# feiyeha/BS-YOLO

Hardware: AMD Instinct MI355X
Metric: images/sec YOLO11s 640x640 bs=64 (forward + NMS) (higher is better)
Workload: dtype f16

## Files before the change

### bs_yolo_amd/csrc/common.h

```cpp
#pragma once
#include <hip/hip_runtime.h>
#include <stdint.h>
#include <stdio.h>
#include <string>

#include "../../include/bsyolo.h"

typedef _Float16 half_t;
typedef _Float16 half8 __attribute__((ext_vector_type(8)));
typedef _Float16 half4 __attribute__((ext_vector_type(4)));
typedef _Float16 half2v __attribute__((ext_vector_type(2)));
typedef float f32x16 __attribute__((ext_vector_type(16)));
typedef float f32x4 __attribute__((ext_vector_type(4)));

void bsy_set_error(const char* fmt, ...);
#define BSY_FAIL(code, ...)        \
    do {                           \
        bsy_set_error(__VA_ARGS__); \
        return (code);             \
    } while (0)
#define HIP_TRY(expr)                                                                                     \
    do {                                                                                                  \
        hipError_t _e = (expr);                                                                           \
        if (_e != hipSuccess) BSY_FAIL(BSY_ERR_HIP, "%s failed: %s (%s:%d)", #expr, hipGetErrorString(_e), \
                                       __FILE__, __LINE__);                                               \
    } while (0)

static inline int ceil_div(int a, int b) { return (a + b - 1) / b; }
static inline int round_up(int a, int b) { return ceil_div(a, b) * b; }

struct ConvArgs {
    const half_t* src0;
    const half_t* src1;
    int ld0, ld1;
    int C0, C1;
    int up0, up1;
    int B, H, W, OH, OW;
    int ksize, stride, pad;
    const half_t* wgt;
    const float* bias;
    void* dst;
    int ldd, Cout, out_f32;
    const half_t* res;
    int ldr;
    int act;
    int dst_scale, dst_dy, dst_dx;
    int cfg;
    int epi;
    void* y;
    int y_f32, A, a0, nrows;
    float lvl_stride;
    void* raw;
    int raw_f32, rawC;
    const half_t* tail_wgt;
    const float* tail_bias;
    int nsl_c = 0, nsl_t = 0;
    float* split_ws = nullptr;
};
int launch_conv(const ConvArgs& a, hipStream_t s);
#define BSY_CONV_MAX_CFG 64
int conv_candidates(const ConvArgs& a, int* out, int max_out);
bool conv_cfg_valid(const ConvArgs& a, int cfg);
int conv_korder(const ConvArgs& a);

struct ConvFirstArgs {
    const void* img;
    int img_dtype;
    int B, H, W, OH, OW, ksize, stride, pad;
    const void* w;
    const float* b;
    half_t* dst;
    int ldd, Cout, act;
};
int launch_conv_first(const ConvFirstArgs& a, hipStream_t s);

struct StemArgs {
    const void* img;
    int img_dtype;
    int B, H, W, OH, OW;
    const void* w0;
    const float* b0;
    const void* w1;
    const float* b1;
    int C0, C1, Kpad1;
    half_t* dst;
    int ldd, act;
};
bool stem_fused_supported(int C0, int C1, int H, int W);
int launch_stem_fused(const StemArgs& a, hipStream_t s);

struct BneckArgs {
    const half_t* src;
    int lds;
    int B, H, W, C, CH;
    const void *w1, *w2;
    const float *b1, *b2;
    int Kpad1, Kpad2;
    half_t* dst;
    int ldd, act;
};
bool bneck_fused_supported(int C, int CH);
int launch_bneck_fused(const BneckArgs& a, hipStream_t s);

struct C3k2Args {
    const half_t* src;
    int lds;
    int B, H, W, Cin, C, C2;
    const void *w1, *wa, *wb, *w4;
    const float *b1, *ba, *bb, *b4;
    half_t* dst;
    int ldd;
};
bool c3k2_fused_supported(int Cin, int C, int C2);
int launch_c3k2_fused(const C3k2Args& a, hipStream_t s);

struct DwGenArgs {
    const half_t* src;
    int lds;
    int B, H, W, C, OH, OW, kh, kw, stride;
    const float* w;
    int wld;
    const float* b;
    half_t* dst;
    int ldd, act_c;
    int ident_c0 = 0;
};
int launch_dwconv_generic(const DwGenArgs& a, hipStream_t s);
struct PmsfaArgs {
    const half_t* P;
    int ldp;
    const half_t* x;
    int ldx;
    half_t* dst;
    int ldd;
    int B, H, W, C;
    const float* w2;
    const float* b2;
    int wld2;
    const float* w3;
    const float* b3;
// ... 290 lines not shown
```

### bs_yolo_amd/csrc/conv_gemm.hip

```cpp
#include "conv_kernels.h"


__device__ __attribute__((aligned(16))) unsigned int bsy_zero_page[16];

template <int KS, int WAVES_M, int WAVES_N, int MT, int NT, int STAGES, bool ALIGNED, int BK>
__global__ __launch_bounds__(64 * WAVES_M * WAVES_N) void conv_mfma_kernel(const ConvK p) {
    constexpr int NW = WAVES_M * WAVES_N;
    constexpr int NTHR = 64 * NW;
    static_assert(BK == 32 || (BK == 64 && ALIGNED), "BK = 64 only for aligned layers");
    constexpr int TM = WAVES_M * MT * 32;
    constexpr int TN = WAVES_N * NT * 32;
    constexpr int TNS = TN < 64 ? 64 : TN;
    constexpr int CPR = BK / 8;
    constexpr int RPI = 64 / CPR;
    constexpr int PIW = TM / (RPI * NW);
    constexpr int WIW = TNS / (RPI * NW);
    static_assert(PIW >= 1 && WIW >= 1 && (BK == 32 || (!(PIW & 1) && !(WIW & 1))), "tile too small for this wave count");
    constexpr int STAGE = (TM + TNS) * BK;
    constexpr int NDMA = PIW + WIW;
    constexpr int SWS = BK == 32 ? 2 : 1;
    constexpr int OTILE = (TM > TN ? TM : TN) * ((TM > TN ? TN : TM) + 8);
    constexpr int SMEM = STAGES * STAGE > OTILE ? STAGES * STAGE : OTILE;
    __shared__ __attribute__((aligned(16))) half_t smem[SMEM];

    const int tid = threadIdx.x;
    const int lane = tid & 63;
    const int wave = __builtin_amdgcn_readfirstlane(tid >> 6);
    const int wm = wave / WAVES_N, wn = wave % WAVES_N;
    int wg = xcd_remap(blockIdx.x, gridDim.x);
    const bool split = ALIGNED && p.nsl_c * p.nsl_t > 1;
    int slice = 0;
    if (split) {
        const int per = p.ntn * ((p.M + TM - 1) / TM);
        slice = wg / per;
        wg -= slice * per;
    }
    const int tap0 = split ? (slice % p.nsl_t) * p.taps_per : 0, tap1 = split ? tap0 + p.taps_per : p.ntaps;
    const int cb0 = split ? (slice / p.nsl_t) * p.cb_per : 0, cb1 = split ? cb0 + p.cb_per : p.Cin8 * 8;
    const int tn_idx = wg % p.ntn;
    const int tm_idx = wg / p.ntn;
    const int m0 = tm_idx * TM;
    const int n0 = tn_idx * TN;

    const int rsub = lane / CPR;
    const int slot = lane % CPR;
    const int kc0 = BK == 32 ? (slot ^ ((rsub >> 2) & 3)) : (slot ^ (rsub >> 1));
    const int kc1 = BK == 32 ? kc0 : (slot ^ (4 | (rsub >> 1)));
    unsigned off0[PIW], off1[PIW], vmask[PIW];
    const int ohw = p.OH * p.OW;
#pragma unroll
    for (int i = 0; i < PIW; ++i) {
        const int m = m0 + (wave * PIW + i) * RPI + rsub;
        const bool rv = m < p.M;
        const int mm = rv ? m : 0;
        int n, oh, ow;
        if (KS == 1 && p.stride == 1) {
            n = 0; oh = 0; ow = 0;
            if (p.up0 | p.up1) { n = mm / ohw; const int rem = mm - n * ohw; oh = rem / p.OW; ow = rem - oh * p.OW; }
        } else {
            n = mm / ohw; const int rem = mm - n * ohw; oh = rem / p.OW; ow = rem - oh * p.OW;
        }
        const int iy0 = oh * p.stride - p.pad, ix0 = ow * p.stride - p.pad;
        if (KS == 1) {
            vmask[i] = rv ? 1u : 0u;
            if (p.stride == 1 && !(p.up0 | p.up1)) {
                off0[i] = (unsigned)mm * (unsigned)p.ld0;
                off1[i] = (unsigned)mm * (unsigned)p.ld1;
            } else {
                const int H0 = p.H >> p.up0, W0 = p.W >> p.up0, H1 = p.H >> p.up1, W1 = p.W >> p.up1;
                off0[i] = (unsigned)((n * H0 + (iy0 >> p.up0)) * W0 + (ix0 >> p.up0)) * (unsigned)p.ld0;
                off1[i] = (unsigned)((n * H1 + (iy0 >> p.up1)) * W1 + (ix0 >> p.up1)) * (unsigned)p.ld1;
            }
        } else {
            unsigned rb = 0, cb = 0;
#pragma unroll
            for (int t = 0; t < KS; ++t) {
                rb |= ((unsigned)(iy0 + t) < (unsigned)p.H ? 1u : 0u) << t;
                cb |= ((unsigned)(ix0 + t) < (unsigned)p.W ? 1u : 0u) << t;
            }
            unsigned vm = 0;
#pragma unroll
            for (int t = 0; t < KS; ++t) vm |= ((rb >> t) & 1u) ? (cb << (t * KS)) : 0u;
            vmask[i] = rv ? vm : 0u;
            const unsigned pix = (unsigned)((n * p.H + iy0) * p.W + ix0);
            off0[i] = pix * (unsigned)p.ld0;
            off1[i] = pix * (unsigned)p.ld1;
        }
    }
    unsigned woff[WIW];
#pragma unroll
    for (int j = 0; j < WIW; ++j)
    {
        const int wrow = min(n0 + (wave * WIW + j) * RPI + rsub, ((p.Cout + 127) & ~127) - 1);
        woff[j] = (unsigned)wrow * (unsigned)p.Kpad + ((j & 1) ? kc1 : kc0) * 8;
    }
    const half_t* zero = reinterpret_cast<const half_t*>(bsy_zero_page);
    const bsy_rsrc_t rs0 = make_rsrc(p.src0, p.span0), rs1 = make_rsrc(p.src1 ? p.src1 : p.src0, p.src1 ? p.span1 : 0u),
                     rsw = make_rsrc(p.wgt, p.wspan);

    int s_tap = tap0, s_cb = cb0;
    int tap = ALIGNED ? 0 : kc0 / p.Cin8;
    int c8 = ALIGNED ? 0 : kc0 - tap * p.Cin8;
    const int Cin = p.Cin8 * 8;

    auto issue = [&](int kt, int stage, const int s_tap, const int s_cb, const int tap, const int c8) {
        half_t* sP = smem + stage * STAGE;
        half_t* sW = sP + TM * BK;
#ifdef BSY_ABLATE
        if (BSY_ABLATE & 1) return;
#endif
        if (ALIGNED) {
            const bool s1 = s_cb >= p.C0;
            const int ld = s1 ? p.ld1 : p.ld0;
            const int kh = (KS == 1) ? 0 : s_tap / KS;
            const int kw = (KS == 1) ? 0 : s_tap - kh * KS;
            const unsigned sc = 2u * (unsigned)((kh * p.W + kw) * ld + (s1 ? s_cb - p.C0 : s_cb));
            const unsigned tbit = 1u << s_tap;
#pragma unroll
            for (int i = 0; i < PIW; ++i) {
                const unsigned kcb = 16u * (unsigned)((i & 1) ? kc1 : kc0);
                const unsigned o = (vmask[i] & tbit) ? 2u * (s1 ? off1[i] : off0[i]) + sc + kcb : BSY_OOB;
                if (s1) dma16_buf(rs1, o, 0u, sP + (wave * PIW + i) * RPI * BK);
                else dma16_buf(rs0, o, 0u, sP + (wave * PIW + i) * RPI * BK);
            }
#pragma unroll
            for (int j = 0; j < WIW; ++j)
                dma16_buf(rsw, 2u * woff[j], 2u * (unsigned)(s_tap * Cin + s_cb), sW + (wave * WIW + j) * RPI * BK);
        } else {
            const bool kvalid = tap < p.ntaps;
            const int kh = (KS == 1) ? 0 : tap / KS;
            const int kw = (KS == 1) ? 0 : tap - kh * KS;
            const int cc = c8 * 8;
            const bool s1 = cc >= p.C0;
            const half_t* base = s1 ? p.src1 : p.src0;
            const int ld = s1 ? p.ld1 : p.ld0;
            const unsigned sc = (unsigned)((kh * p.W + kw) * ld + (s1 ? cc - p.C0 : cc));
            const unsigned tbit = kvalid ? (1u << tap) : 0u;
#pragma unroll
            for (int i = 0; i < PIW; ++i) {
                const unsigned o = (s1 ? off1[i] : off0[i]) + sc;
                const half_t* g = (vmask[i] & tbit) ? base + (size_t)o : zero;
                dma16(g, sP + (wave * PIW + i) * RPI * BK);
            }
#pragma unroll
            for (int j = 0; j < WIW; ++j)
                dma16(p.wgt + (size_t)(woff[j] + (unsigned)kt * 32u), sW + (wave * WIW + j) * RPI * BK);
        }
    };
#define BSY_ADVANCE_K()                                                                                  \
    do {                                                                                                 \
        if (ALIGNED) {                                                                                   \
            if (p.korder == 1 || (p.korder == 2 && BK == 64)) {  \
                if (++s_tap >= tap1) { s_tap = tap0; s_cb += BK; }                                       \
            } else if (p.korder == 2) {        \
                if (s_cb & 32) { s_cb -= 32; if (++s_tap >= tap1) { s_tap = tap0; s_cb += 64; } }        \
                else s_cb += 32;                                                                         \
            } else {                                                                                     \
                s_cb += BK;                                                                              \
                if (s_cb >= cb1) { s_cb = cb0; ++s_tap; }                                                \
            }                                                                                            \
        } else {                                                                                         \
            c8 += 4;                                                                                     \
            while (c8 >= p.Cin8) { c8 -= p.Cin8; ++tap; }                                                \
        }                                                                                                \
    } while (0)

    const int lrow = lane & 31;
    const int lh = lane >> 5;
    const int nk = split ? (tap1 - tap0) * (cb1 - cb0) / BK : p.Kpad / BK;
    f32x16 acc[NT][MT];
#pragma unroll
    for (int a = 0; a < NT; ++a)
#pragma unroll
        for (int b = 0; b < MT; ++b) {
            acc_bias(acc[a][b], p.bias + n0 + (wn * NT + a) * 32, lh);
            if (slice) {
#pragma unroll
                for (int r = 0; r < 16; ++r) acc[a][b][r] = 0.f;
            }
        }

#pragma unroll
    for (int s = 0; s < STAGES - 1; ++s)
        if (s < nk) { issue(s, s, s_tap, s_cb, tap, c8); BSY_ADVANCE_K(); }

    for (int kt = 0; kt < nk; ++kt) {
        const int later = min(STAGES - 2, nk - 1 - kt);
        if (later >= STAGES - 2 && STAGES > 2) {
            asm volatile("s_waitcnt vmcnt(%0)" ::"n"((STAGES - 2) * NDMA) : "memory");
        } else if (STAGES > 3 && later == STAGES - 3) {
            asm volatile("s_waitcnt vmcnt(%0)" ::"n"((STAGES > 3 ? STAGES - 3 : 0) * NDMA) : "memory");
        } else {
            asm volatile("s_waitcnt vmcnt(0)" ::: "memory");
        }
        __builtin_amdgcn_s_barrier();
        if (kt + STAGES - 1 < nk) { issue(kt + STAGES - 1, (kt + STAGES - 1) % STAGES, s_tap, s_cb, tap, c8); BSY_ADVANCE_K(); }
        const half_t* sP = smem + (kt % STAGES) * STAGE;
        const half_t* sW = sP + TM * BK;
        constexpr int KSUB = BK / 16;
        half8 bfr[2][MT], afr[2][NT];
        auto rd = [&](const int ks, const int buf) {
            const int chunk = 2 * ks + lh;
#pragma unroll
            for (int b = 0; b < MT; ++b) {
                const int row = (wm * MT + b) * 32 + lrow;
                bfr[buf][b] = *reinterpret_cast<const half8*>(sP + row * BK + ((chunk ^ ((row >> SWS) & (CPR - 1))) << 3));
            }
#pragma unroll
            for (int a = 0; a < NT; ++a) {
                const int row = (wn * NT + a) * 32 + lrow;
                afr[buf][a] = *reinterpret_cast<const half8*>(sW + row * BK + ((chunk ^ ((row >> SWS) & (CPR - 1))) << 3));
            }
        };
        rd(0, 0);
#pragma unroll
        for (int ks = 0; ks < KSUB; ++ks) {
            if (ks + 1 < KSUB) rd(ks + 1, (ks + 1) & 1);
            __builtin_amdgcn_sched_barrier(0);
#pragma unroll
            for (int a = 0; a < NT; ++a)
#pragma unroll
                for (int b = 0; b < MT; ++b)
                    acc[a][b] = __builtin_amdgcn_mfma_f32_32x32x16_f16(afr[ks & 1][a], bfr[ks & 1][b], acc[a][b], 0, 0, 0);
            __builtin_amdgcn_sched_barrier(0);
        }
    }
#ifdef BSY_ABLATE
    if (BSY_ABLATE & 4) {
        if (acc[0][0][0] == 12345.678f) reinterpret_cast<float*>(p.dst)[0] = 1.f;
        return;
    }
#endif
    if (split) {
        float* ws = p.split_ws + (size_t)slice * (size_t)p.slab;
#pragma unroll
        for (int b = 0; b < MT; ++b) {
            const int m = m0 + (wm * MT + b) * 32 + lrow;
            if (m >= p.M) continue;
#pragma unroll
            for (int a = 0; a < NT; ++a) {
                const int cbase = n0 + (wn * NT + a) * 32;
#pragma unroll
                for (int g = 0; g < 4; ++g) {
                    const int c = cbase + 8 * g + 4 * lh;
                    if (c < p.ldw) *reinterpret_cast<f32x4*>(ws + (size_t)m * p.ldw + c) = f32x4{acc[a][b][4 * g], acc[a][b][4 * g + 1], acc[a][b][4 * g + 2], acc[a][b][4 * g + 3]};
                }
            }
        }
        return;
    }
    if (p.epi) {
        if (p.epi == 2 && !p.y_f32 && !p.raw) {
            __syncthreads();
            conv_epilogue_cls_lds<TM, TN, MT, NT, NTHR>(p, acc, smem, m0, n0, wm, wn, lrow, lh, tid);
        } else {
            conv_epilogue_head<MT, NT>(p, acc, m0, n0, wm, wn, lrow, lh);
        }
        return;
    }
    const bool lds_epi = !p.out_f32 && !(p.Cout & 7) && !(p.ldd & 7) && !((uintptr_t)p.dst & 15) && p.dst_scale == 1 &&
                         (!p.res || (!(p.ldr & 7) && !((uintptr_t)p.res & 15)));
    if (lds_epi) {
        __syncthreads();
        conv_epilogue_lds<TM, TN, MT, NT, NTHR>(p, acc, smem, m0, n0, wm, wn, lrow, lh, tid);
    } else {
        conv_epilogue<MT, NT>(p, acc, m0, n0, wm, wn, lrow, lh);
    }
}

#undef BSY_ADVANCE_K

__global__ __launch_bounds__(256) void splitk_reduce_kernel(const float* __restrict__ ws, const int nsl, const long long slab, const int ldw,
                                                           const int M, const int Cout, const int act, const half_t* __restrict__ res, const int ldr,
                                                           half_t* __restrict__ dst, const int ldd) {
    const int c8n = Cout >> 3;
    const long long idx = (long long)blockIdx.x * 256 + threadIdx.x;
    if (idx >= (long long)M * c8n) return;
    const int c = (int)(idx % c8n) * 8;
    const size_t m = (size_t)(idx / c8n);
    const float* wp = ws + m * ldw + c;
    f32x4 a0 = *reinterpret_cast<const f32x4*>(wp), a1 = *reinterpret_cast<const f32x4*>(wp + 4);
    for (int sl = 1; sl < nsl; ++sl) {
        const float* q = wp + (size_t)sl * (size_t)slab;
        a0 = add4_f(a0, *reinterpret_cast<const f32x4*>(q));
        a1 = add4_f(a1, *reinterpret_cast<const f32x4*>(q + 4));
    }
    float v[8] = {a0[0], a0[1], a0[2], a0[3], a1[0], a1[1], a1[2], a1[3]};
    if (act) {
#pragma unroll
        for (int e = 0; e < 8; ++e) v[e] = silu_f(v[e]);
    }
    if (res) {
        const half8 rv = *reinterpret_cast<const half8*>(res + m * ldr + c);
#pragma unroll
        for (int e = 0; e < 8; ++e) v[e] += (float)rv[e];
    }
    half8 o;
#pragma unroll
    for (int e = 0; e < 8; ++e) o[e] = (half_t)v[e];
    *reinterpret_cast<half8*>(dst + m * ldd + c) = o;
}

template <int KS, int WM, int WN, int MT, int NT, int STAGES, bool ALIGNED, int BK>
static int launch_cfg(const ConvK& k, hipStream_t s) {
    constexpr int TM = WM * MT * 32, TN = WN * NT * 32;
    ConvK p = k;
    p.ntn = ceil_div(k.Cout, TN);
    const int nsl = k.nsl_c * k.nsl_t;
    const long long nblk = (long long)ceil_div(k.M, TM) * p.ntn * (nsl > 1 ? nsl : 1);
    if (nblk <= 0 || nblk > 0x7fffffffLL) BSY_FAIL(BSY_ERR_ARG, "conv: grid %lld out of range", nblk);
    hipLaunchKernelGGL((conv_mfma_kernel<KS, WM, WN, MT, NT, STAGES, ALIGNED, BK>), dim3((unsigned)nblk), dim3(64 * WM * WN), 0, s, p);
    HIP_TRY(hipGetLastError());
    if (nsl > 1) {
        const long long items = (long long)k.M * (k.Cout >> 3);
        hipLaunchKernelGGL(splitk_reduce_kernel, dim3((unsigned)((items + 255) / 256)), dim3(256), 0, s, k.split_ws, nsl, k.slab, k.ldw, k.M, k.Cout, k.act,
                           k.res, k.ldr, reinterpret_cast<half_t*>(k.dst), k.ldd);
        HIP_TRY(hipGetLastError());
    }
    return BSY_OK;
}

template <int WM, int WN, int MT, int NT, int S, bool AL, int BK>
static int launch_gemm(int ksize, const ConvK& k, hipStream_t s) {
    return ksize == 3 ? launch_cfg<3, WM, WN, MT, NT, S, AL, BK>(k, s) : launch_cfg<1, WM, WN, MT, NT, S, AL, BK>(k, s);
}

int launch_gemm_cfg(int id, int ksize, const ConvK& k, hipStream_t s) {
    switch (id) {
        case 0x00: return launch_gemm<4, 1, 2, 1, 3, false, 32>(ksize, k, s);
        case 0x01: return launch_gemm<4, 1, 2, 1, 3, true, 32>(ksize, k, s);
        case 0x02: return launch_gemm<4, 1, 2, 1, 2, true, 32>(ksize, k, s);
        case 0x03: return launch_gemm<4, 1, 2, 1, 2, true, 64>(ksize, k, s);
        case 0x10: return launch_gemm<4, 1, 2, 2, 3, false, 32>(ksize, k, s);
        case 0x11: return launch_gemm<4, 1, 2, 2, 3, true, 32>(ksize, k, s);
        case 0x12: return launch_gemm<4, 1, 2, 2, 2, true, 32>(ksize, k, s);
        case 0x13: return launch_gemm<4, 1, 2, 2, 2, true, 64>(ksize, k, s);
        case 0x20: return launch_gemm<2, 2, 2, 2, 3, false, 32>(ksize, k, s);
        case 0x21: return launch_gemm<2, 2, 2, 2, 3, true, 32>(ksize, k, s);
        case 0x22: return launch_gemm<2, 2, 2, 2, 2, true, 32>(ksize, k, s);
        case 0x23: return launch_gemm<2, 2, 2, 2, 2, true, 64>(ksize, k, s);
        case 0x30: return launch_gemm<2, 2, 2, 1, 3, false, 32>(ksize, k, s);
        case 0x31: return launch_gemm<2, 2, 2, 1, 3, true, 32>(ksize, k, s);
        case 0x32: return launch_gemm<2, 2, 2, 1, 2, true, 32>(ksize, k, s);
        case 0x33: return launch_gemm<2, 2, 2, 1, 2, true, 64>(ksize, k, s);
        case 0x41: return launch_gemm<4, 2, 2, 2, 3, true, 32>(ksize, k, s);
        case 0x42: return launch_gemm<4, 2, 2, 2, 2, true, 32>(ksize, k, s);
        case 0x43: return launch_gemm<4, 2, 2, 2, 2, true, 64>(ksize, k, s);
        case 0x50: return launch_gemm<1, 4, 2, 1, 3, false, 32>(ksize, k, s);
        case 0x51: return launch_gemm<1, 4, 2, 1, 3, true, 32>(ksize, k, s);
        case 0x52: return launch_gemm<1, 4, 2, 1, 2, true, 32>(ksize, k, s);
        case 0x53: return launch_gemm<1, 4, 2, 1, 2, true, 64>(ksize, k, s);
        case 0x60: return launch_gemm<2, 2, 1, 1, 3, false, 32>(ksize, k, s);
        case 0x61: return launch_gemm<2, 2, 1, 1, 3, true, 32>(ksize, k, s);
        case 0x62: return launch_gemm<2, 2, 1, 1, 2, true, 32>(ksize, k, s);
        case 0x63: return launch_gemm<2, 2, 1, 1, 2, true, 64>(ksize, k, s);
        case 0x71: return launch_gemm<4, 2, 2, 4, 3, true, 32>(ksize, k, s);
        case 0x72: return launch_gemm<4, 2, 2, 4, 2, true, 32>(ksize, k, s);
        case 0x73: return launch_gemm<4, 2, 2, 4, 2, true, 64>(ksize, k, s);
    }
    BSY_FAIL(BSY_ERR_ARG, "conv: no implicit-GEMM kernel is built for configuration 0x%02x", id);
}
```

### bs_yolo_amd/csrc/conv_kernels.h

```cpp
#pragma once
#include "common.h"

struct ConvK {
    const half_t* src0;
    const half_t* src1;
    int ld0, ld1, C0, C1, up0, up1;
    int H, W, OH, OW, stride, pad;
    int M;
    int Cin8;
    int ntaps;
    int nk;
    int Kpad;
    const half_t* wgt;
    const float* bias;
    void* dst;
    int ldd, Cout, out_f32;
    const half_t* res;
    int ldr;
    int act;
    int dst_scale, dst_dy, dst_dx;
    int ntn;
    int ntm;
    int tiles_x, tiles_y, B;
    int epi, y_f32, A, a0, nrows, raw_f32, rawC;
    float lvl_stride;
    void* y;
    void* raw;
    const half_t* tail_wgt;
    const float* tail_bias;
    unsigned span0, span1, wspan;
    int nsl_c, nsl_t, cb_per, taps_per, ldw;
    float* split_ws;
    long long slab;
    int korder;
};

__device__ __forceinline__ void dma16(const void* g, half_t* lds_wave_base) {
#if defined(__HIP_DEVICE_COMPILE__)
    __builtin_amdgcn_global_load_lds(g, lds_wave_base, 16, 0, 0);
#else
    (void)g;
    (void)lds_wave_base;
#endif
}

#if defined(__HIP_DEVICE_COMPILE__)
__device__ __forceinline__ void dma16_buf(bsy_rsrc_t r, unsigned voff, unsigned soff, half_t* lds_wave_base) {
    __builtin_amdgcn_raw_ptr_buffer_load_lds(r, lds_wave_base, 16, (int)voff, (int)soff, 0, 0);
}
#else
__device__ __forceinline__ void dma16_buf(bsy_rsrc_t, unsigned, unsigned, half_t*) {}
#endif

template <int MT, int NT>
__device__ __forceinline__ void conv_epilogue(const ConvK& p, f32x16 (&acc)[NT][MT], int m0, int n0, int wm, int wn,
                                              int lrow, int lh) {
    const int ohw = p.OH * p.OW;
    const bool wide = !p.out_f32 && !(p.Cout & 15) && !(p.ldd & 7) && !((uintptr_t)p.dst & 15);
#pragma unroll
    for (int b = 0; b < MT; ++b) {
        const int m = m0 + (wm * MT + b) * 32 + lrow;
        const bool mvalid = m < p.M;
        size_t dpix = (size_t)(mvalid ? m : 0);
        if (p.dst_scale != 1) {
            const int mm = mvalid ? m : 0;
            const int n = mm / ohw;
            const int rem = mm - n * ohw;
            const int oh = rem / p.OW;
            const int ow = rem - oh * p.OW;
            dpix = ((size_t)n * (p.OH * p.dst_scale) + (oh * p.dst_scale + p.dst_dy)) * (size_t)(p.OW * p.dst_scale) +
                   (ow * p.dst_scale + p.dst_dx);
        }
#pragma unroll
        for (int a = 0; a < NT; ++a) {
            const int cbase = n0 + (wn * NT + a) * 32;
            if (cbase >= p.Cout) continue;
            if (wide) {
                unsigned pk[4][2];
#pragma unroll
                for (int g = 0; g < 4; ++g) {
                    const int c = cbase + 8 * g + 4 * lh;
                    float v[4] = {0.f, 0.f, 0.f, 0.f};
                    if (c < p.Cout) {
#pragma unroll
                        for (int e = 0; e < 4; ++e) {
                            float t = acc[a][b][4 * g + e];
                            v[e] = p.act ? silu_f(t) : t;
                        }
                        if (p.res && mvalid) {
                            const half4 rv = *reinterpret_cast<const half4*>(p.res + dpix * p.ldr + c);
#pragma unroll
                            for (int e = 0; e < 4; ++e) v[e] += (float)rv[e];
                        }
                    }
                    half2v h0 = {(half_t)v[0], (half_t)v[1]}, h1 = {(half_t)v[2], (half_t)v[3]};
                    pk[g][0] = __builtin_bit_cast(unsigned, h0);
                    pk[g][1] = __builtin_bit_cast(unsigned, h1);
                }
#pragma unroll
                for (int g = 0; g < 4; g += 2) {
                    const auto r0 = __builtin_amdgcn_permlane32_swap(pk[g][0], pk[g + 1][0], false, false);
                    const auto r1 = __builtin_amdgcn_permlane32_swap(pk[g][1], pk[g + 1][1], false, false);
                    const int c = cbase + 8 * (g + lh);
                    if (mvalid && c < p.Cout) {
                        uint4 o = {r0[0], r1[0], r0[1], r1[1]};
                        *reinterpret_cast<uint4*>(reinterpret_cast<half_t*>(p.dst) + dpix * p.ldd + c) = o;
                    }
                }
                continue;
            }
            if (!mvalid) continue;
#pragma unroll
            for (int g = 0; g < 4; ++g) {
                const int c = cbase + 8 * g + 4 * lh;
                if (c >= p.Cout) continue;
                float v[4];
#pragma unroll
// ... 138 lines not shown
                                                      int wm, int wn, int lrow, int lh, int tid) {
    constexpr int LDP = TM + 8;
#pragma unroll
    for (int b = 0; b < MT; ++b) {
        const int prow = (wm * MT + b) * 32 + lrow;
#pragma unroll
        for (int a = 0; a < NT; ++a) {
            const int cl = (wn * NT + a) * 32;
            if (n0 + cl >= p.Cout) continue;
#pragma unroll
            for (int g = 0; g < 4; ++g) {
                const int c = cl + 8 * g + 4 * lh;
#pragma unroll
                for (int e = 0; e < 4; ++e) {
                    const float v = acc[a][b][4 * g + e];
                    stile[(c + e) * LDP + prow] = (half_t)sigmoid_f(v);
                }
            }
        }
    }
    __syncthreads();
    const int hw = p.OH * p.OW;
    half_t* y = reinterpret_cast<half_t*>(p.y);
    constexpr int GPR = TM / 8;
    for (int id = tid; id < TN * GPR; id += NTHR) {
        const int cr = id / GPR, g8 = (id - cr * GPR) * 8;
        const int c = n0 + cr, m = m0 + g8;
        if (c >= p.Cout || m >= p.M) continue;
        const int n = m / hw, pix = m - n * hw;
        const size_t yi = ((size_t)n * p.nrows + 4 + c) * p.A + p.a0 + pix;
        if (pix + 8 <= hw && m + 8 <= p.M && !(yi & 7)) {
            *reinterpret_cast<half8*>(y + yi) = *reinterpret_cast<const half8*>(stile + cr * LDP + g8);
        } else {
            for (int e = 0; e < 8 && m + e < p.M; ++e) {
                const int me = m + e, ne = me / hw, pe = me - ne * hw;
                y[((size_t)ne * p.nrows + 4 + c) * p.A + p.a0 + pe] = stile[cr * LDP + g8 + e];
            }
        }
    }
}

template <int TM, int TN, int MT, int NT, int NTHR>
__device__ __forceinline__ void conv_epilogue_lds(const ConvK& p, f32x16 (&acc)[NT][MT], half_t* stile, int m0, int n0,
                                                  int wm, int wn, int lrow, int lh, int tid) {
    constexpr int LDT = TN + 8;
#pragma unroll
    for (int b = 0; b < MT; ++b) {
        const int prow = (wm * MT + b) * 32 + lrow;
#pragma unroll
        for (int a = 0; a < NT; ++a) {
            const int cl = (wn * NT + a) * 32;
#pragma unroll
            for (int g = 0; g < 4; ++g) {
                const int c = cl + 8 * g + 4 * lh;
                half4 o;
                f32x4 t = f32x4{acc[a][b][4 * g], acc[a][b][4 * g + 1], acc[a][b][4 * g + 2], acc[a][b][4 * g + 3]};
                if (p.act) t = silu4_f(t);
#pragma unroll
                for (int e = 0; e < 4; ++e) o[e] = (half_t)t[e];
                *reinterpret_cast<half4*>(stile + prow * LDT + c) = o;
            }
        }
    }
    __syncthreads();
    constexpr int CPRW = TN / 8;
    constexpr int ITER = TM * CPRW / NTHR;
    half_t* dst = reinterpret_cast<half_t*>(p.dst);
#pragma unroll
    for (int i = 0; i < ITER; ++i) {
        const int id = tid + NTHR * i;
        const int row = id / CPRW, cc = (id % CPRW) * 8;
        const int m = m0 + row, c = n0 + cc;
        if (m >= p.M || c >= p.Cout) continue;
        half8 v = *reinterpret_cast<const half8*>(stile + row * LDT + cc);
        if (p.res) {
            const half8 r = *reinterpret_cast<const half8*>(p.res + (size_t)m * p.ldr + c);
#pragma unroll
            for (int e = 0; e < 8; ++e) v[e] = (half_t)((float)v[e] + (float)r[e]);
        }
        *reinterpret_cast<half8*>(dst + (size_t)m * p.ldd + c) = v;
    }
}

int launch_gemm_cfg(int id, int ksize, const ConvK& k, hipStream_t s);
int launch_stream1x1_cfg(int id, const ConvK& k, hipStream_t s);
int launch_patch_cfg(int id, bool tail, const ConvK& k, hipStream_t s);

constexpr int PERSIST_MAX_COUT = 1024;
```

### bs_yolo_amd/csrc/conv_select.hip

```cpp
#include <stdlib.h>

#include "conv_kernels.h"

extern "C" int bsy_conv_packed_dims(int C2, int C1, int ksize, int* cout_pad, int* k_pad) {
    if (C2 <= 0 || C1 <= 0 || (ksize != 1 && ksize != 3)) BSY_FAIL(BSY_ERR_ARG, "conv_packed_dims: bad shape");
    if (cout_pad) *cout_pad = round_up(C2, 128);
    if (C1 == 3) C1 = 4;
    if (k_pad) *k_pad = round_up(ksize * ksize * C1, 32);
    return BSY_OK;
}

int conv_korder(const ConvArgs& a) {
    const int Cin = a.C0 + a.C1;
    if (a.ksize != 3 || (Cin & 31) || (a.C0 & 31)) return 0;
    return (a.stride == 2 && !(Cin & 63) && !(a.C0 & 63)) ? 2 : 1;
}

enum ConvFam { CONV_GEMM, CONV_PERSIST, CONV_WRES, CONV_PATCH, CONV_TAIL };
struct ConvCfg {
    int id; ConvFam fam;
    int tm, tn, stages, bk;
    bool aligned;
    int tw, nfr;
};
template <int WM, int WN, int MT, int NT, int S, bool AL, int BK> constexpr ConvCfg gemm_row(int id) {
    return {id, CONV_GEMM, WM * MT * 32, WN * NT * 32, S, BK, AL, 0, 0};
}
template <int WM, int WN, int MT, int NT, int S, int BK> constexpr ConvCfg persist_row(int id) {
    return {id, CONV_PERSIST, WM * MT * 32, WN * NT * 32, S, BK, true, 0, 0};
}
template <int NT, int S, int NFR> constexpr ConvCfg wres_row(int id) {
    return {id, CONV_WRES, 128, 64 * NT, S, 32, true, 0, NFR};
}
template <int NT, int S, int TW, bool TAIL = false> constexpr ConvCfg patch_row(int id) {
    return {id, TAIL ? CONV_TAIL : CONV_PATCH, TW == 16 ? 8 * 16 : 6 * 20, 64 * NT, S, 32, true, TW, 0};
}
static const ConvCfg kConvCfgs[] = {
    gemm_row<4, 1, 2, 1, 3, false, 32>(0x00),
    gemm_row<4, 1, 2, 1, 3, true, 32>(0x01),
    gemm_row<4, 1, 2, 1, 2, true, 32>(0x02),
    gemm_row<4, 1, 2, 1, 2, true, 64>(0x03),
    gemm_row<4, 1, 2, 2, 3, false, 32>(0x10),
    gemm_row<4, 1, 2, 2, 3, true, 32>(0x11),
    gemm_row<4, 1, 2, 2, 2, true, 32>(0x12),
    gemm_row<4, 1, 2, 2, 2, true, 64>(0x13),
    gemm_row<2, 2, 2, 2, 3, false, 32>(0x20),
    gemm_row<2, 2, 2, 2, 3, true, 32>(0x21),
    gemm_row<2, 2, 2, 2, 2, true, 32>(0x22),
    gemm_row<2, 2, 2, 2, 2, true, 64>(0x23),
    gemm_row<2, 2, 2, 1, 3, false, 32>(0x30),
    gemm_row<2, 2, 2, 1, 3, true, 32>(0x31),
    gemm_row<2, 2, 2, 1, 2, true, 32>(0x32),
    gemm_row<2, 2, 2, 1, 2, true, 64>(0x33),
    gemm_row<4, 2, 2, 2, 3, true, 32>(0x41),
    gemm_row<4, 2, 2, 2, 2, true, 32>(0x42),
    gemm_row<4, 2, 2, 2, 2, true, 64>(0x43),
    gemm_row<1, 4, 2, 1, 3, false, 32>(0x50),
    gemm_row<1, 4, 2, 1, 3, true, 32>(0x51),
    gemm_row<1, 4, 2, 1, 2, true, 32>(0x52),
    gemm_row<1, 4, 2, 1, 2, true, 64>(0x53),
    gemm_row<2, 2, 1, 1, 3, false, 32>(0x60),
    gemm_row<2, 2, 1, 1, 3, true, 32>(0x61),
    gemm_row<2, 2, 1, 1, 2, true, 32>(0x62),
    gemm_row<2, 2, 1, 1, 2, true, 64>(0x63),
    gemm_row<4, 2, 2, 4, 3, true, 32>(0x71),
    gemm_row<4, 2, 2, 4, 2, true, 32>(0x72),
    gemm_row<4, 2, 2, 4, 2, true, 64>(0x73),
    persist_row<2, 2, 2, 2, 3, 32>(0x81),
    persist_row<2, 2, 2, 2, 2, 32>(0x82),
    persist_row<2, 2, 2, 2, 2, 64>(0x83),
    persist_row<2, 2, 2, 1, 3, 32>(0x91),
    persist_row<2, 2, 2, 1, 2, 32>(0x92),
    persist_row<2, 2, 2, 1, 2, 64>(0x93),
    patch_row<2, 2, 16>(0xA1),
    patch_row<1, 3, 16>(0xB1),
    patch_row<1, 2, 16>(0xB2),
    patch_row<1, 4, 16>(0xB3),
    patch_row<2, 2, 20>(0xC1),
    patch_row<1, 3, 20>(0xD1),
    patch_row<1, 2, 20>(0xD2),
    patch_row<1, 4, 20>(0xD3),
    patch_row<1, 3, 16, true>(0xB1),
    patch_row<1, 2, 16, true>(0xB2),
    patch_row<1, 4, 16, true>(0xB3),
    patch_row<1, 3, 20, true>(0xD1),
    patch_row<1, 2, 20, true>(0xD2),
    patch_row<1, 4, 20, true>(0xD3),
    wres_row<2, 4, 24>(0xE1),
    wres_row<2, 3, 24>(0xE2),
    wres_row<1, 4, 32>(0xF1),
    wres_row<1, 3, 32>(0xF2),
};

static const ConvCfg* conv_cfg_row(int cfg, bool tail) {
    for (const ConvCfg& r : kConvCfgs) if (r.id == (cfg & ~4) && (r.fam == CONV_TAIL) == tail) return &r;
    return nullptr;
}

bool conv_cfg_valid(const ConvArgs& a, int cfg) {
    const ConvCfg* r = conv_cfg_row(cfg, a.tail_wgt != nullptr);
    if (!r) return false;
    const int Cin = a.C0 + a.C1, ko = conv_korder(a), nsl = a.nsl_c * a.nsl_t;
    const bool aligned = !(Cin & 31) && !(a.C0 & 31), aligned64 = !(Cin & 63) && !(a.C0 & 63);
    if ((r->aligned && !aligned) || (r->bk == 64 && !aligned64)) return false;
    if (r->fam == CONV_GEMM) {
        if (!(cfg & 4) != !ko) return false;
        if (ko && (!r->aligned || (ko == 1 && r->bk == 64))) return false;
        if (nsl > 1 && (!r->aligned || (Cin / (a.nsl_c > 0 ? a.nsl_c : 1)) % r->bk)) return false;
        if (a.epi == 3 && (r->tm != 256 || r->tn != 64)) return false;
        return r->tn != 256 || !(a.Cout & 255);
    }
    if ((cfg & 4) || nsl > 1 || (r->fam == CONV_TAIL ? (a.epi != 3 || a.Cout != 64 || a.res) : a.epi != 0)) return false;
    if (a.out_f32 || (a.Cout & 7) || (a.ldd & 7) || ((uintptr_t)a.dst & 15) || a.dst_scale > 1) return false;
    if (r->fam == CONV_PERSIST || r->fam == CONV_WRES) {
        if (a.ksize != 1 || a.stride != 1 || a.res) return false;
        if (r->fam == CONV_PERSIST) return a.Cout <= PERSIST_MAX_COUT;
        return (r->tn / 64) * (Cin / 16) <= r->nfr && Cin / 32 >= r->stages - 1 && (r->tn != 128 || a.Cout > 64);
    }
    return ko == 1 && a.ksize == 3 && a.stride == 1 && a.pad == 1 && !a.C1 && !a.up0 && (!a.res || (!(a.ldr & 7) && !((uintptr_t)a.res & 15))) &&
           (r->tn != 128 || a.Cout > 64);
}

static bool family_off(const char* env) { return getenv(env) != nullptr; }

int conv_candidates(const ConvArgs& a, int* out, int max_out) {
    const int Cin = a.C0 + a.C1;
    const bool aligned = !(Cin & 31) && !(a.C0 & 31), aligned64 = !(Cin & 63) && !(a.C0 & 63);
    const long long M = (long long)a.B * a.OH * a.OW;
    const int tile = a.epi == 3 ? 1 : (a.Cout > 64 ? 2 : (a.Cout > 32 ? 1 : 0));
    const int ko = conv_korder(a), km = ko ? 4 : 0;
    const bool t20 = ceil_div(a.W, 20) * ceil_div(a.H, 6) < ceil_div(a.W, 16) * ceil_div(a.H, 8);
    int n = 0;
    auto add = [&](int c) {
        for (int i = 0; i < n; ++i) if (out[i] == c) return;
        if (n < max_out && conv_cfg_valid(a, c)) out[n++] = c;
    };
    if (a.tail_wgt) {
        if (t20) { add(0xD2); add(0xD1); add(0xD3); }
        add(0xB2); add(0xB1); add(0xB3); add(0xD2); add(0xD1); add(0xD3);
        return n;
    }
    if (!aligned) {
        add(tile << 4);
        if (a.Cout > 32) { add(0x30); add(0x60); }
        if (a.Cout > 64) add(0x50);
        return n;
    }
    const bool patch_ok = !family_off("BSY_NO_PATCH");
    if (!a.epi && a.ksize == 3 && a.stride == 1 && a.H >= 16 && a.W >= 16 && patch_ok) add(t20 ? 0xD2 : 0xB2);
    const int vbest = (aligned64 && ko != 1) ? 3 : 1;
    if (!a.epi && !(a.Cout & 255) && aligned64 && ko != 1 && M >= 16384) add(0x73 | km);
    add(tile << 4 | vbest | km);
    for (const ConvCfg& r : kConvCfgs) {
        if ((r.fam != CONV_GEMM && r.fam != CONV_PERSIST) || !r.aligned) continue;
        if (r.tn >= 2 * round_up(a.Cout, 32)) continue;
        if (r.tn == 32 && a.Cout > 32) continue;
        if (r.tm == 256 && r.tn == 128 && (a.Cout < 128 || M < 32768)) continue;
        if (r.tn == 256 && M < 16384) continue;
        if (r.fam == CONV_PERSIST && (M < 65536 || family_off("BSY_NO_PERSIST"))) continue;
        add(r.id | (r.fam == CONV_GEMM ? km : 0));
    }
    if (a.ksize == 1 && M >= 65536 && !family_off("BSY_NO_WRES"))
        for (const ConvCfg& r : kConvCfgs) if (r.fam == CONV_WRES) add(r.id);
    if (a.H >= 16 && a.W >= 16 && patch_ok)
        for (const ConvCfg& r : kConvCfgs) if (r.fam == CONV_PATCH && (r.tw == 16 || t20)) add(r.id);
    return n;
}

int launch_conv(const ConvArgs& a, hipStream_t s) {
    const int Cin = a.C0 + a.C1;
    if (a.ksize != 1 && a.ksize != 3) BSY_FAIL(BSY_ERR_ARG, "conv: ksize %d unsupported", a.ksize);
    if (a.stride != 1 && a.stride != 2) BSY_FAIL(BSY_ERR_ARG, "conv: stride %d unsupported", a.stride);
    if ((a.C0 & 7) || (a.C1 & 7) || (a.ld0 & 7) || (a.C1 && (a.ld1 & 7)))
        BSY_FAIL(BSY_ERR_ARG, "conv: channel counts/strides must be multiples of 8 (C0=%d C1=%d ld0=%d ld1=%d)", a.C0,
                 a.C1, a.ld0, a.ld1);
    if ((a.ldd & 3) || (a.res && (a.ldr & 3))) BSY_FAIL(BSY_ERR_ARG, "conv: dst/res row stride must be a multiple of 4");
    if (((uintptr_t)a.src0 & 15) || ((uintptr_t)a.src1 & 15) || ((uintptr_t)a.wgt & 15) || ((uintptr_t)a.bias & 15) ||
        ((uintptr_t)a.dst & 7) || ((uintptr_t)a.res & 7))
        BSY_FAIL(BSY_ERR_ARG, "conv: misaligned pointer");
    if (a.C1 && !a.src1) BSY_FAIL(BSY_ERR_ARG, "conv: src1 missing");
    if ((a.up0 && ((a.H | a.W) & 1)) || (a.up1 && ((a.H | a.W) & 1))) BSY_FAIL(BSY_ERR_ARG, "conv: odd size with upsample");
    if (a.OH != (a.H + 2 * a.pad - a.ksize) / a.stride + 1 || a.OW != (a.W + 2 * a.pad - a.ksize) / a.stride + 1)
        BSY_FAIL(BSY_ERR_ARG, "conv: output extent mismatch");
    const long long M = (long long)a.B * a.OH * a.OW;
    if (M <= 0 || M > 0x7fffffffLL) BSY_FAIL(BSY_ERR_ARG, "conv: M out of range");
    if (a.epi) {
        if ((a.epi != 2 && a.epi != 3) || !a.y || a.A <= 0 || a.a0 < 0 || a.a0 + a.OH * a.OW > a.A || a.dst_scale > 1 || a.res)
            BSY_FAIL(BSY_ERR_ARG, "conv: bad fused-decoder arguments (epi %d)", a.epi);
        if (a.epi == 3 && (a.Cout != 64 || a.nrows < 4)) BSY_FAIL(BSY_ERR_ARG, "conv: DFL epilogue needs 64 box channels");
        if (a.tail_wgt && (a.epi != 3 || !a.tail_bias || a.ksize != 3 || ((uintptr_t)a.tail_wgt & 15) || ((uintptr_t)a.tail_bias & 15)))
            BSY_FAIL(BSY_ERR_ARG, "conv: bad box-branch tail arguments");
        if (a.epi == 2 && a.nrows < 4 + a.Cout) BSY_FAIL(BSY_ERR_ARG, "conv: y has %d rows, class epilogue needs %d", a.nrows, 4 + a.Cout);
        if (a.raw && a.rawC < (a.epi == 3 ? 64 : 64 + a.Cout)) BSY_FAIL(BSY_ERR_ARG, "conv: raw map has too few channels");
    }
    ConvK k;
    k.src0 = a.src0; k.src1 = a.src1; k.ld0 = a.ld0; k.ld1 = a.ld1; k.C0 = a.C0; k.C1 = a.C1;
    k.up0 = a.up0; k.up1 = a.up1; k.H = a.H; k.W = a.W; k.OH = a.OH; k.OW = a.OW; k.stride = a.stride; k.pad = a.pad;
    k.M = (int)M; k.Cin8 = Cin / 8; k.ntaps = a.ksize * a.ksize;
    k.Kpad = round_up(a.ksize * a.ksize * Cin, 32); k.nk = k.Kpad / 32;
    k.wgt = a.wgt; k.bias = a.bias; k.dst = a.dst; k.ldd = a.ldd; k.Cout = a.Cout; k.out_f32 = a.out_f32;
    k.res = a.res; k.ldr = a.ldr; k.act = a.act; k.B = a.B; k.tiles_x = k.tiles_y = 0;
    k.epi = a.epi; k.y = a.y; k.y_f32 = a.y_f32; k.A = a.A; k.a0 = a.a0; k.nrows = a.nrows; k.lvl_stride = a.lvl_stride;
    k.raw = a.raw; k.raw_f32 = a.raw_f32; k.rawC = a.rawC;
    k.tail_wgt = a.tail_wgt; k.tail_bias = a.tail_bias;
    if (a.tail_wgt && !a.epi) BSY_FAIL(BSY_ERR_ARG, "conv: a box-branch tail needs the decoder arguments (epi 3)");
    k.dst_scale = a.dst_scale > 0 ? a.dst_scale : 1; k.dst_dy = a.dst_dy; k.dst_dx = a.dst_dx; k.ntn = 1;
    k.nsl_c = k.nsl_t = 1; k.cb_per = Cin; k.taps_per = a.ksize * a.ksize; k.split_ws = nullptr; k.slab = 0; k.ldw = 0;
    if (a.nsl_c * a.nsl_t > 1) {
        const int nt = a.ksize * a.ksize;
        if (a.nsl_c < 1 || a.nsl_t < 1 || !a.split_ws || a.epi || a.out_f32 || a.tail_wgt || (a.dst_scale > 1) || (Cin % a.nsl_c) || ((Cin / a.nsl_c) & 31) || (a.C0 & 31) ||
            (nt % a.nsl_t) || (a.Cout & 7) || (a.ldd & 7) || ((uintptr_t)a.dst & 15) || (a.res && ((a.ldr & 7) || ((uintptr_t)a.res & 15))) || ((uintptr_t)a.split_ws & 15))
            BSY_FAIL(BSY_ERR_ARG, "conv: bad split-K arguments (%d x %d slices)", a.nsl_c, a.nsl_t);
        if (conv_korder(a) == 2 && ((Cin / a.nsl_c) & 63)) BSY_FAIL(BSY_ERR_ARG, "conv: split-K slices of a 64-channel-chunk layer must be multiples of 64 channels");
        k.nsl_c = a.nsl_c; k.nsl_t = a.nsl_t; k.cb_per = Cin / a.nsl_c; k.taps_per = nt / a.nsl_t; k.split_ws = a.split_ws;
        k.ldw = round_up(a.Cout, 32);
        k.slab = (long long)M * k.ldw;
    }
    if (a.ksize == 3 && (a.up0 || a.up1)) BSY_FAIL(BSY_ERR_ARG, "conv: upsampled source only with ksize 1");
    if ((long long)a.B * a.H * a.W * (long long)(a.ld0 > a.ld1 ? a.ld0 : a.ld1) >= (1LL << 31))
        BSY_FAIL(BSY_ERR_ARG, "conv: source view exceeds 2^31 elements (split the batch)");
    {
        const long long px0 = (long long)a.B * (a.H >> a.up0) * (a.W >> a.up0), px1 = (long long)a.B * (a.H >> a.up1) * (a.W >> a.up1);
        k.span0 = (unsigned)(((px0 - 1) * a.ld0 + a.C0) * 2);
        k.span1 = a.C1 ? (unsigned)(((px1 - 1) * a.ld1 + a.C1) * 2) : 0u;
        k.wspan = (unsigned)((long long)round_up(a.Cout, 128) * k.Kpad * 2);
    }
    int cfg = a.cfg;
    if (cfg < 0 || !conv_cfg_valid(a, cfg)) {
        int list[BSY_CONV_MAX_CFG];
        if (conv_candidates(a, list, BSY_CONV_MAX_CFG) <= 0) BSY_FAIL(BSY_ERR_ARG, "conv: no kernel configuration for this shape");
        cfg = list[0];
    }
    k.korder = conv_korder(a);
    const ConvCfg* r = conv_cfg_row(cfg, a.tail_wgt != nullptr);
    switch (r->fam) {
        case CONV_GEMM: return launch_gemm_cfg(r->id, a.ksize, k, s);
        case CONV_PERSIST:
        case CONV_WRES: return launch_stream1x1_cfg(r->id, k, s);
        case CONV_PATCH:
        case CONV_TAIL: return launch_patch_cfg(r->id, r->fam == CONV_TAIL, k, s);
    }
    BSY_FAIL(BSY_ERR_ARG, "conv: configuration 0x%02x has no kernel family", cfg);
}
```

### bs_yolo_amd/csrc/engine.hip

```cpp
#include <stdlib.h>
#include <string.h>

#include <algorithm>
#include <vector>

#include "common.h"
#include "postproc.h"

struct bsy_engine {
    int device = 0;
    void* weights = nullptr;
    size_t weight_bytes = 0;
    char* arena = nullptr;
    size_t arena_bytes = 0;
    unsigned arena_gen = 0;
    unsigned weights_gen = 0;
};

struct bsy_plan {
    bsy_engine* eng = nullptr;
    std::vector<bsy_op> ops;
    std::vector<size_t> buf_off;
    std::vector<size_t> buf_size;
    char* workspace = nullptr;
// ... 416 lines not shown
            return launch_pmsfa_tail(a, s);
        }
        case BSY_OP_COPY: {
            const half_t* src = R.h(op.src0);
            half_t* dst = R.h(op.dst);
            if (!R.ok) return BSY_ERR_ARG;
            return launch_copy_view(src, op.src0.ld, op.up0, op.B, op.H, op.W, op.src0.C, dst, op.dst.ld, s);
        }
        case BSY_OP_GAP: {
            const half_t* src = R.h(op.src0);
            half_t* dst = R.h(op.dst);
            if (!R.ok) return BSY_ERR_ARG;
            return launch_gap(src, op.src0.ld, op.B, op.H, op.W, op.src0.C, dst, op.dst.ld, s);
        }
        case BSY_OP_MSCA_SPATIAL: {
            MscaSpArgs a;
            a.src = R.h(op.src0); a.lds = op.src0.ld; a.B = op.B; a.H = op.H; a.W = op.W; a.C = op.src0.C;
            for (int i = 0; i < 9; ++i) {
                a.w[i] = (const float*)(wb + op.aux_off[2 * i]);
                a.b[i] = (const float*)(wb + op.aux_off[2 * i + 1]);
            }
            for (int i = 0; i < 4; ++i) {
                const bsy_view& bv = i < 3 ? op.box[i] : op.res;
                const bsy_view& gv = i < 3 ? op.cls[i] : op.msk[0];
                a.br[i] = R.h(bv); a.ldb[i] = bv.ld; a.gap[i] = R.h(gv); a.ldg[i] = gv.ld;
            }
            if (!R.ok) return BSY_ERR_ARG;
            return launch_msca_spatial(a, s);
        }
        case BSY_OP_MSCA_MIX: {
            MixArgs a;
            for (int i = 0; i < 4; ++i) {
                const bsy_view& bv = i < 3 ? op.box[i] : op.res;
                const bsy_view& lv = i < 3 ? op.cls[i] : op.msk[0];
                a.br[i] = R.h(bv); a.ldb[i] = bv.ld; a.lg[i] = R.f(lv); a.ldl[i] = lv.ld;
            }
            a.B = op.B; a.HW = op.H * op.W; a.C = op.dst.C; a.dst = R.h(op.dst); a.ldd = op.dst.ld;
            if (!R.ok) return BSY_ERR_ARG;
            return launch_msca_mix(a, s);
        }
        case BSY_OP_MUL: {
            const half_t* x = R.h(op.src0);
            const half_t* y = R.h(op.src1);
            half_t* dst = R.h(op.dst);
            if (!R.ok) return BSY_ERR_ARG;
            return launch_mul(x, op.src0.ld, y, op.src1.ld, (long long)op.B * op.H * op.W, op.dst.C, dst, op.dst.ld, s);
        }
        case BSY_OP_ELA: {
            ElaArgs a;
            a.src = R.h(op.src0); a.lds = op.src0.ld; a.B = op.B; a.H = op.H; a.W = op.W; a.C = op.src0.C; a.k = op.ksize;
            const float* blob = (const float*)(wb + op.w_off);
            a.wsp = blob; a.wch = blob + (size_t)a.C * a.k; a.gnw = a.wch + (size_t)a.C * a.k; a.gnb = a.gnw + a.C;
            a.ch_coef = op.scale; a.sp_coef = op.lvl_stride[0]; a.res_coef = op.lvl_stride[1];
            a.scratch = R.f(op.res); a.dst = R.h(op.dst); a.ldd = op.dst.ld;
            if (!R.ok) return BSY_ERR_ARG;
            return launch_ela(a, s);
        }
        case BSY_OP_CONV: {
            ConvArgs a;
            a.src0 = R.h(op.src0); a.src1 = R.h(op.src1);
            a.ld0 = op.src0.ld; a.ld1 = op.src1.buf >= 0 ? op.src1.ld : 0;
            a.C0 = op.src0.C; a.C1 = op.src1.buf >= 0 ? op.src1.C : 0;
            a.up0 = op.up0; a.up1 = op.up1;
            a.B = op.B; a.H = op.H; a.W = op.W; a.OH = op.OH; a.OW = op.OW;
            a.ksize = op.ksize; a.stride = op.stride; a.pad = op.pad;
            a.wgt = (const half_t*)(wb + op.w_off); a.bias = (const float*)(wb + op.b_off);
            a.dst = op.out_f32 ? (void*)R.f(op.dst) : (void*)R.h(op.dst);
            a.ldd = op.dst.ld; a.Cout = op.dst.C; a.out_f32 = op.out_f32;
            a.res = R.h(op.res); a.ldr = op.res.buf >= 0 ? op.res.ld : 0;
            a.act = op.act; a.dst_scale = op.dst_scale; a.dst_dy = op.dst_dy; a.dst_dx = op.dst_dx;
            a.epi = 0; a.y = nullptr; a.raw = nullptr; a.y_f32 = a.raw_f32 = a.A = a.a0 = a.nrows = a.rawC = 0; a.lvl_stride = 0.f;
            a.tail_wgt = nullptr; a.tail_bias = nullptr;
            if (op.out_f32 >= 2) {
                a.epi = op.out_f32; a.out_f32 = 0; a.dst = nullptr; a.ldd = 8; a.Cout = op.nl;
                a.y = R.base(op.dst); a.y_f32 = op.out_dtype == BSY_F32; a.A = op.A; a.a0 = op.lvl_h[1]; a.nrows = op.dst.C;
                a.lvl_stride = op.lvl_stride[0];
                const bsy_view& rv = op.box[0];
                const bool bound = rv.buf >= BSY_EXT_BASE && rv.buf - BSY_EXT_BASE < R.n_ext && R.ext[rv.buf - BSY_EXT_BASE];
                a.raw = bound ? R.base(rv) : nullptr; a.raw_f32 = a.y_f32; a.rawC = rv.C;
                if (op.out_f32 == 3 && op.mid_c > 0) {
                    a.Cout = op.mid_c;
                    a.tail_wgt = (const half_t*)(wb + op.w2_off); a.tail_bias = (const float*)(wb + op.b2_off);
                }
            }
            if (op.ksplit > 0 && op.out_f32 == 0) {
                a.nsl_c = op.ksplit & 255; a.nsl_t = (op.ksplit >> 8) & 255;
                a.split_ws = R.f(op.box[0]);
            }
            a.cfg = op.tuned_cfg - 1;
            if (!R.ok) return BSY_ERR_ARG;
            if (cargs) { *cargs = a; return BSY_OK; }
            return launch_conv(a, s);
        }
        case BSY_OP_DWCONV: {
            DwArgs a;
            a.src = R.h(op.src0); a.lds = op.src0.ld; a.B = op.B; a.H = op.H; a.W = op.W; a.C = op.src0.C;
            a.w = (const float*)(wb + op.w_off); a.b = (const float*)(wb + op.b_off);
            a.dst = R.h(op.dst); a.ldd = op.dst.ld; a.act = op.act;
            a.res = R.h(op.res); a.ldr = op.res.buf >= 0 ? op.res.ld : 0;
            if (!R.ok) return BSY_ERR_ARG;
            return launch_dwconv(a, s);
        }
        case BSY_OP_SPPF_POOL: {
            half_t* b = R.h(op.src0);
            if (!R.ok) return BSY_ERR_ARG;
            return launch_sppf_pool(b, op.src0.ld, op.B, op.H, op.W, op.src0.C, s);
        }
        case BSY_OP_ATTN: {
            AttnArgs a;
            a.qkv = R.h(op.src0); a.ld = op.src0.ld; a.B = op.B; a.N = op.H * op.W; a.heads = op.heads;
            a.key_dim = op.key_dim; a.head_dim = op.head_dim; a.scale = op.scale;
            a.out = R.h(op.dst); a.ldo = op.dst.ld;
            if (!R.ok) return BSY_ERR_ARG;
            return launch_attention(a, s);
        }
        case BSY_OP_DECODE: {
            DecodeArgs a;
            memset(&a, 0, sizeof(a));
            a.nl = op.nl; a.B = op.B; a.nc = op.nc; a.nm = op.nm; a.A = op.A; a.ne = op.ne;
            const bool extra = op.nm || op.ne;
            for (int l = 0; l < op.nl && l < BSY_MAX_LEVELS; ++l) {
                a.box[l] = R.f(op.box[l]); a.cls[l] = R.f(op.cls[l]); a.msk[l] = extra ? R.f(op.msk[l]) : nullptr;
                a.ldb[l] = op.box[l].ld; a.ldc[l] = op.cls[l].ld; a.ldm[l] = extra ? op.msk[l].ld : 0;
                a.h[l] = op.lvl_h[l]; a.w[l] = op.lvl_w[l]; a.stride[l] = op.lvl_stride[l];
            }
            a.y = R.base(op.dst); a.y_dtype = op.out_dtype;
            if (!R.ok) return BSY_ERR_ARG;
            return launch_decode(a, s);
        }
        case BSY_OP_RAW_NCHW: {
            const int l = op.level;
            if (l < 0 || l >= BSY_MAX_LEVELS) BSY_FAIL(BSY_ERR_ARG, "raw_nchw: level %d", l);
            if (op.dst.buf >= BSY_EXT_BASE && (op.dst.buf - BSY_EXT_BASE >= R.n_ext || !R.ext[op.dst.buf - BSY_EXT_BASE]))
                return BSY_OK;
            const float* box = R.f(op.box[l]);
            const float* cls = R.f(op.cls[l]);
            void* out = R.base(op.dst);
            if (!R.ok) return BSY_ERR_ARG;
            return launch_raw_nchw(box, op.box[l].ld, cls, op.cls[l].ld, op.B, op.lvl_h[l], op.lvl_w[l], op.nc, out,
                                   op.out_dtype, s);
        }
        case BSY_OP_NHWC2NCHW: {
            if (op.dst.buf >= BSY_EXT_BASE && (op.dst.buf - BSY_EXT_BASE >= R.n_ext || !R.ext[op.dst.buf - BSY_EXT_BASE]))
                return BSY_OK;
            const half_t* src = R.h(op.src0);
            void* out = R.base(op.dst);
            if (!R.ok) return BSY_ERR_ARG;
            return launch_nhwc2nchw(src, op.src0.ld, op.B, op.src0.C, op.H * op.W, out, op.out_dtype, s);
        }
        default:
            BSY_FAIL(BSY_ERR_ARG, "plan_run: unknown op kind %d", op.kind);
    }
}
}

extern "C" void bsy_plan_destroy(bsy_plan* p);

extern "C" int bsy_plan_run(bsy_plan* p, void* const* ext, int n_ext, bsy_stream stream) {
    if (!p || (n_ext && !ext)) BSY_FAIL(BSY_ERR_ARG, "plan_run: bad argument");
    hipStream_t main = (hipStream_t)stream;
    Resolver R{p, ext, n_ext};
    unsigned active = 0;
    int rc = BSY_OK;
    for (size_t i = 0; i < p->ops.size() && rc == BSY_OK; ++i) {
        const bsy_op& op = p->ops[i];
        if (op.join && active) {
// ... 178 lines not shown
    }
    for (size_t i = 0; i < NCAL; ++i) HIP_TRY(hipEventRecord(p->events[n + 1 + i], s));
    HIP_TRY(hipEventSynchronize(p->events[n + NCAL]));
    float cal[NCAL];
    for (size_t i = 0; i < NCAL; ++i) HIP_TRY(hipEventElapsedTime(&cal[i], p->events[n + i], p->events[n + 1 + i]));
    std::sort(cal, cal + NCAL);
    const float ev_ms = cal[NCAL / 2];
    for (size_t i = 0; i < n; ++i) {
        HIP_TRY(hipEventElapsedTime(&ms_per_op[i], p->events[i], p->events[i + 1]));
        ms_per_op[i] = ms_per_op[i] > ev_ms ? ms_per_op[i] - ev_ms : 0.f;
    }
    p->last_event_overhead_ms = ev_ms;
    return BSY_OK;
}

extern "C" int bsy_plan_autotune_in_place(bsy_plan* p, void* const* ext, int n_ext, bsy_stream stream, int rounds) {
    if (!p || (n_ext && !ext) || rounds < 1 || rounds > 16) BSY_FAIL(BSY_ERR_ARG, "plan_autotune_in_place: bad argument");
    p->drop_graphs();
    hipStream_t s = (hipStream_t)stream;
    const size_t n = p->ops.size();
    Resolver R{p, ext, n_ext};
    std::vector<std::vector<int>> cand(n);
    size_t K = 0;
    for (size_t i = 0; i < n; ++i) {
        bsy_op& op = p->ops[i];
        if (op.kind == BSY_OP_CONV && op.tuned_cfg <= 0 && op.prec == 0) {
            ConvArgs a;
            int rc = run_op(p, op, R, s, &a);
            if (rc != BSY_OK) return rc;
            int list[BSY_CONV_MAX_CFG];
            const int nc = conv_candidates(a, list, BSY_CONV_MAX_CFG);
            cand[i].assign(list, list + (nc > 0 ? nc : 0));
            K = cand[i].size() > K ? cand[i].size() : K;
        }
        const int rc = run_op(p, op, R, s);
        if (rc != BSY_OK) return rc;
    }
    if (K == 0) return BSY_OK;
    std::vector<float> best(n, 1e30f), ms(n);
    std::vector<std::vector<float>> tk(n);
    for (size_t i = 0; i < n; ++i) tk[i].assign(cand[i].size(), 1e30f);
    std::vector<int> best_c(n, -1);
    for (size_t i = 0; i < n; ++i)
        if (!cand[i].empty()) best_c[i] = cand[i][0];
    for (size_t k = 0; k < K; ++k) {
        for (size_t i = 0; i < n; ++i)
            if (!cand[i].empty()) p->ops[i].tuned_cfg = (k < cand[i].size() ? cand[i][k] : best_c[i]) + 1;
        for (int r = 0; r < rounds; ++r) {
            const int rc = bsy_plan_profile(p, ext, n_ext, stream, ms.data());
            if (rc != BSY_OK) {
                for (size_t i = 0; i < n; ++i)
                    if (!cand[i].empty()) p->ops[i].tuned_cfg = 0;
                return rc;
            }
            for (size_t i = 0; i < n; ++i)
                if (k < cand[i].size()) {
                    if (ms[i] < tk[i][k]) tk[i][k] = ms[i];
                    if (ms[i] < best[i]) { best[i] = ms[i]; best_c[i] = cand[i][k]; }
                }
        }
    }
    for (size_t i = 0; i < n; ++i)
        if (!cand[i].empty()) p->ops[i].tuned_cfg = best_c[i] + 1;
    return BSY_OK;
}

extern "C" int bsy_conv2d(const void* x, int ldx, int B, int H, int W, int C1, const void* w, const float* b, void* y,
                          int ldy, int C2, int ksize, int stride, int act, const void* res, int ldr, int y_f32,
                          bsy_stream stream) {
    if (!x || !w || !b || !y) BSY_FAIL(BSY_ERR_ARG, "conv2d: null pointer");
    ConvArgs a;
    memset(&a, 0, sizeof(a));
    a.src0 = (const half_t*)x; a.ld0 = ldx; a.C0 = C1; a.B = B; a.H = H; a.W = W;
    a.ksize = ksize; a.stride = stride; a.pad = ksize / 2;
    a.OH = (H + 2 * a.pad - ksize) / stride + 1; a.OW = (W + 2 * a.pad - ksize) / stride + 1;
    a.wgt = (const half_t*)w; a.bias = b; a.dst = y; a.ldd = ldy; a.Cout = C2; a.out_f32 = y_f32;
    a.res = (const half_t*)res; a.ldr = ldr; a.act = act; a.dst_scale = 1;
    const char* forced = getenv("BSY_CONV_CFG");
    a.cfg = forced ? atoi(forced) : -1;
    if (a.cfg >= 0 && !conv_cfg_valid(a, a.cfg)) BSY_FAIL(BSY_ERR_ARG, "conv: BSY_CONV_CFG=%d is not valid for this shape", a.cfg);
    return launch_conv(a, (hipStream_t)stream);
}

extern "C" int bsy_conv2d_f32(const float* x, int ldx, int B, int H, int W, int C1, const float* w, const float* b, float* y, int ldy,
                              int C2, int ksize, int stride, int act, const float* res, int ldr, int impl, bsy_stream stream) {
    if (!x || !w || !b || !y) BSY_FAIL(BSY_ERR_ARG, "conv2d_f32: null pointer");
    if (B <= 0 || H <= 0 || W <= 0 || C1 <= 0 || C2 <= 0 || ksize < 1 || !(ksize & 1) || (stride != 1 && stride != 2) || ldx < C1 || ldy < C2 ||
        (res && ldr < C2) || impl < 0 || impl > 2)
        BSY_FAIL(BSY_ERR_ARG, "conv2d_f32: bad shape");
    Conv32Args a;
    memset(&a, 0, sizeof(a));
    a.src0 = x; a.src_dtype = BSY_F32; a.ld0 = ldx; a.C0 = C1; a.B = B; a.H = H; a.W = W;
    a.ks = ksize; a.stride = stride; a.pad = ksize / 2;
    a.OH = (H + 2 * a.pad - ksize) / stride + 1; a.OW = (W + 2 * a.pad - ksize) / stride + 1;
    a.w = w; a.bias = b; a.dst = y; a.ldd = ldy; a.Cout = C2; a.res = res; a.ldr = ldr; a.act = act; a.dst_scale = 1;
    if (impl == 1) return launch_conv32_scalar(a, (hipStream_t)stream);
    if (impl == 2) return launch_conv32_mfma(a, (hipStream_t)stream);
    return launch_conv32(a, (hipStream_t)stream);
}

extern "C" int bsy_conv2d_f32x(const float* x, int ldx, int B, int H, int W, int C1, const void* w_hi, const void* w_lo, int k_pad,
                               const float* b, float* y, int ldy, int C2, int ksize, int stride, int act, const float* res, int ldr,
                               bsy_stream stream) {
    if (!x || !w_hi || !w_lo || !b || !y) BSY_FAIL(BSY_ERR_ARG, "conv2d_f32x: null pointer");
    if (B <= 0 || H <= 0 || W <= 0 || C1 <= 0 || C2 <= 0 || ksize < 1 || !(ksize & 1) || (stride != 1 && stride != 2) || ldx < C1 || ldy < C2 ||
        (res && ldr < C2) || k_pad < ksize * ksize * C1 || (k_pad & 31))
        BSY_FAIL(BSY_ERR_ARG, "conv2d_f32x: bad shape");
    Conv32Args a;
    memset(&a, 0, sizeof(a));
    a.src0 = x; a.src_dtype = BSY_F32; a.ld0 = ldx; a.C0 = C1; a.B = B; a.H = H; a.W = W;
    a.ks = ksize; a.stride = stride; a.pad = ksize / 2;
    a.OH = (H + 2 * a.pad - ksize) / stride + 1; a.OW = (W + 2 * a.pad - ksize) / stride + 1;
    a.w = (const float*)w_hi;
    a.bias = b; a.dst = y; a.ldd = ldy; a.Cout = C2; a.res = res; a.ldr = ldr; a.act = act; a.dst_scale = 1;
    a.wx_hi = (const half_t*)w_hi; a.wx_lo = (const half_t*)w_lo; a.wx_kpad = k_pad;
    return launch_conv32x_mfma(a, (hipStream_t)stream);
}

extern "C" int bsy_conv_first_f32(const void* img, int img_dtype, int B, int H, int W, const float* w, const float* b, float* y, int ldy,
                                 int C2, int ksize, int stride, int act, int impl, bsy_stream stream) {
    if (!img || !w || !b || !y) BSY_FAIL(BSY_ERR_ARG, "conv_first_f32: null pointer");
    if (B <= 0 || H <= 0 || W <= 0 || C2 <= 0 || ksize < 1 || !(ksize & 1) || (stride != 1 && stride != 2) || ldy < C2 || impl < 0 || impl > 2 ||
        (img_dtype != BSY_F16 && img_dtype != BSY_F32))
        BSY_FAIL(BSY_ERR_ARG, "conv_first_f32: bad shape");
    Conv32Args a;
    memset(&a, 0, sizeof(a));
    a.first = 1; a.src0 = img; a.src_dtype = img_dtype; a.C0 = 3; a.B = B; a.H = H; a.W = W;
    a.ks = ksize; a.stride = stride; a.pad = ksize / 2;
    a.OH = (H + 2 * a.pad - ksize) / stride + 1; a.OW = (W + 2 * a.pad - ksize) / stride + 1;
    a.w = w; a.bias = b; a.dst = y; a.ldd = ldy; a.Cout = C2; a.act = act; a.dst_scale = 1;
    if (impl == 1) return launch_conv32_scalar(a, (hipStream_t)stream);
    if (impl == 2) return launch_conv32_mfma(a, (hipStream_t)stream);
    return launch_conv32(a, (hipStream_t)stream);
}

extern "C" int bsy_attention_f32(const float* qkv, int ld, int B, int N, int heads, int key_dim, int head_dim, float scale, float* out,
                                 int ldo, int impl, bsy_stream stream) {
    if (!qkv || !out || B <= 0 || N <= 0 || impl < 0 || impl > 3) BSY_FAIL(BSY_ERR_ARG, "attention_f32: bad argument");
    if (impl == 3) return launch_attn32x(qkv, ld, B, N, heads, key_dim, head_dim, scale, out, ldo, (hipStream_t)stream);
    return launch_attn32(qkv, ld, B, N, heads, key_dim, head_dim, scale, out, ldo, (hipStream_t)stream, impl);
}

extern "C" int bsy_conv_first(const void* img, int img_dtype, int B, int H, int W, const void* w, const float* b,
                              void* y, int ldy, int C2, int ksize, int stride, int act, bsy_stream stream) {
    if (!img || !w || !b || !y) BSY_FAIL(BSY_ERR_ARG, "conv_first: null pointer");
    ConvFirstArgs a;
    a.img = img; a.img_dtype = img_dtype; a.B = B; a.H = H; a.W = W; a.ksize = ksize; a.stride = stride; a.pad = ksize / 2;
    a.OH = (H + 2 * a.pad - ksize) / stride + 1; a.OW = (W + 2 * a.pad - ksize) / stride + 1;
    a.w = w; a.b = b; a.dst = (half_t*)y; a.ldd = ldy; a.Cout = C2; a.act = act;
    return launch_conv_first(a, (hipStream_t)stream);
}

extern "C" int bsy_stem_fused(const void* img, int img_dtype, int B, int H, int W, const void* w0, const float* b0, int C0,
                              const void* w1, const float* b1, int C1, void* y, int ldy, int act, bsy_stream stream) {
    if (!img || !w0 || !b0 || !w1 || !b1 || !y) BSY_FAIL(BSY_ERR_ARG, "stem: null pointer");
    StemArgs a;
    a.img = img; a.img_dtype = img_dtype; a.B = B; a.H = H; a.W = W;
    const int OH0 = (H - 1) / 2 + 1, OW0 = (W - 1) / 2 + 1;
    a.OH = (OH0 - 1) / 2 + 1; a.OW = (OW0 - 1) / 2 + 1;
    a.w0 = w0; a.b0 = b0; a.w1 = w1; a.b1 = b1; a.C0 = C0; a.C1 = C1;
    int cp = 0;
    bsy_conv_packed_dims(C1, C0, 3, &cp, &a.Kpad1);
    a.dst = (half_t*)y; a.ldd = ldy; a.act = act;
    return launch_stem_fused(a, (hipStream_t)stream);
}

// ... 108 lines not shown
```

### bs_yolo_amd/engine.py

```python
from __future__ import annotations

import ctypes as C
import json
import math
import os
from collections import OrderedDict
from typing import Dict, List, Mapping, Optional, Tuple

import torch

from . import lib as L
from . import ops as O
from . import tta as T
from .plan import Plan
from .weights import BN_EPS, adopt_offsets, pack_plan_weights


class YoloEngine:
    def __init__(self, cfg: dict, state_dict: Mapping[str, torch.Tensor], device: int = 0, bn_eps: float = BN_EPS,
                 autotune: Optional[bool] = None, fuse_stem: Optional[bool] = None,
                 fuse_bneck: Optional[bool] = None, fuse_head: Optional[bool] = None, fuse_dwpw: Optional[bool] = None,
                 merge_c3k: Optional[bool] = None, fuse_msca: Optional[bool] = None, fuse_tail: Optional[bool] = None,
                 max_plans: Optional[int] = None, precision: str = "fp16", graph: Optional[bool] = None, graph_ring: int = 3,
                 latency: Optional[bool] = None, fuse_pmsfa: Optional[bool] = None):
        if not torch.cuda.is_available():
            raise RuntimeError("bs_yolo_amd needs a ROCm GPU (there is no CPU fallback)")
        self.cfg = cfg
        self.precision = precision
        self.latency = (os.environ.get("BSY_LATENCY", "0") == "1") if latency is None else bool(latency)
        self.device = torch.device("cuda", device)
        self._h = C.c_void_p()
        L.check(L.lib.bsy_engine_create(device, C.byref(self._h)))
        self._plans: "OrderedDict[Tuple, Tuple]" = OrderedDict()
        self.max_plans = int(os.environ.get("BSY_MAX_PLANS", "8")) if max_plans is None else int(max_plans)
        self._tuned = set()
        self._elems: Dict[Tuple[int, int], int] = {}
        self._tune_cache: Dict[tuple, int] = {}
        self._tune_family: Dict[tuple, int] = {}
        self.tune_stats = {"timed_ops": 0, "cached_ops": 0, "family_ops": 0, "autotune_calls": 0}
        self.tune_mode = os.environ.get("BSY_TUNE_IN_PLACE", "1")
        self._tune_file = os.environ.get("BSY_TUNE_CACHE")
        if self._tune_file and os.path.exists(self._tune_file):
            try:
                self._tune_cache = {tuple(k): int(v) for k, v in json.load(open(self._tune_file))}
                for k, v in self._tune_cache.items():
                    self._tune_family.setdefault(self._family(k), v)
            except (OSError, ValueError):
                self._tune_cache = {}
        self.reuse = os.environ.get("BSY_ARENA_REUSE", "1") != "0" and not os.environ.get("BSY_PLAN_GUARD")
        self.graph = (os.environ.get("BSY_GRAPH", "0") == "1") if graph is None else bool(graph)
        self.graph_ring = max(1, int(graph_ring))
        self._rings: Dict[Tuple, dict] = {}
        self._gstream = None
        import threading
        self._lock = threading.RLock()
        self._last_done = None
        self._last_stream = None
        self.graph_stats = {"captures": 0, "replays": 0, "eager": 0}
        self._tta_geom: Dict[Tuple[int, int], list] = {}
        self._tta_bufs: "OrderedDict[Tuple, torch.Tensor]" = OrderedDict()
        self.autotune = ((os.environ.get("BSY_AUTOTUNE", "1") != "0") if autotune is None else bool(autotune)) and precision == "fp16"
        self.fuse_stem = fuse_stem
        self.fuse_bneck = fuse_bneck
        self.fuse_head = fuse_head
        self.fuse_dwpw = fuse_dwpw
        self.merge_c3k = merge_c3k
        self.fuse_msca = fuse_msca
        self.fuse_tail = fuse_tail
        self.fuse_pmsfa = fuse_pmsfa
        self._packed = Plan(cfg, 1, 64, 64, **self._fuse_kw())
        blob = pack_plan_weights(self._packed, state_dict, bn_eps)
        self.weight_bytes = len(blob)
        buf = (C.c_char * len(blob)).from_buffer_copy(blob)
        L.check(L.lib.bsy_engine_load_weights(self._h, buf, len(blob)))
        self.meta = dict(self._packed.meta)
        self.nc = self.meta["nc"]
        self.stride = torch.tensor(self.meta["strides"])
        self.nl = len(self.meta["levels"])
        self.max_stride = int(max(self.meta["strides"]))
        self.names = {i: f"{i}" for i in range(self.nc)}

    def load_weights(self, state_dict: Mapping[str, torch.Tensor], bn_eps: float = BN_EPS) -> None:
        with self._lock:
            blob = pack_plan_weights(self._packed, state_dict, bn_eps)
            if len(blob) != self.weight_bytes:
                raise ValueError(f"state_dict packs to {len(blob)} bytes, the engine was built for {self.weight_bytes}")
            for plan, _ in self._plans.values():
                adopt_offsets(plan, self._packed)
            buf = (C.c_char * len(blob)).from_buffer_copy(blob)
            L.check(L.lib.bsy_engine_load_weights(self._h, buf, len(blob)))

    def _fuse_kw(self):
        return dict(fuse_stem=self.fuse_stem, fuse_bneck=self.fuse_bneck, fuse_head=self.fuse_head, fuse_dwpw=self.fuse_dwpw,
                    merge_c3k=self.merge_c3k, fuse_msca=self.fuse_msca, fuse_tail=self.fuse_tail, precision=self.precision,
                    lanes=True if getattr(self, "graph", False) else None, latency=getattr(self, "latency", False),
                    fuse_pmsfa=self.fuse_pmsfa)

    def plan_for(self, B: int, H: int, W: int, in_dtype: torch.dtype, out_dtype: torch.dtype):
        key = (B, H, W, in_dtype, out_dtype)
        hit = self._plans.get(key)
        if hit is not None:
            self._plans.move_to_end(key)
            return hit
        gs = self.max_stride
        if H % gs or W % gs:
            raise ValueError(f"input {H}x{W} must be a multiple of the max stride {gs} (utils/checks.py:120-172)")
        plan = Plan(self.cfg, B, H, W, L.dtype_code(in_dtype), L.dtype_code(out_dtype), **self._fuse_kw())
        adopt_offsets(plan, self._packed)
        ops = plan.c_ops()
        sizes = (C.c_int64 * len(plan.buf_bytes))(*plan.buf_bytes)
        h = C.c_void_p()
        with torch.cuda.device(self.device):
            if os.environ.get("BSY_PLAN_GUARD"):
                L.check(L.lib.bsy_plan_create(self._h, ops, len(plan.ops), sizes, len(plan.buf_bytes), C.byref(h)))
                plan.arena_bytes = sum((b + 255) & ~255 for b in plan.buf_bytes)
            else:
                offs, arena = plan.assign_offsets(self.reuse)
                plan.arena_bytes = arena
                L.check(L.lib.bsy_plan_create_arena(self._h, ops, len(plan.ops), sizes, (C.c_int64 * len(offs))(*offs),
                                                    len(offs), arena, C.byref(h)))
        plan.conv_sigs = [plan.conv_signature(o) for o in plan.ops]
        for sg in plan.conv_sigs:
            if sg is not None and sg not in self._tune_cache and self._family(sg) in self._tune_family:
                self._tune_cache[sg] = self._tune_family[self._family(sg)]
                self.tune_stats["family_ops"] += 1
        preset = (C.c_int32 * len(plan.ops))(*[self._tune_cache.get(sg, -1) if sg is not None else -1 for sg in plan.conv_sigs])
        L.check(L.lib.bsy_plan_set_tuning(h, preset, len(plan.ops)))
        while len(self._plans) >= max(self.max_plans, 1):
            old_key, (_, old) = self._plans.popitem(last=False)
            L.lib.bsy_plan_destroy(old)
            for rk in [k for k in self._rings if k[0] == old_key]:
                del self._rings[rk]
        self._plans[key] = (plan, h)
        return plan, h

    @property
    def arena_bytes(self) -> int:
        return int(L.lib.bsy_engine_arena_bytes(self._h))

    @staticmethod
    def _family(sg: tuple) -> tuple:
        B, H, W = sg[:3]
        return sg[3:] + (int(round(math.log2(max(B * H * W, 1)))),)

    def _autotune(self, plan, h, ext, n, stream):
        nops = len(plan.ops)
        valid = (C.c_int32 * nops)()
        L.check(L.lib.bsy_plan_check_tuning(h, ext, n, valid, nops))
        bad = [i for i in range(nops) if valid[i] == 0]
        if bad:
            clear = (C.c_int32 * nops)(*([-1] * nops))
            for i in bad:
                sg = plan.conv_sigs[i]
                cfg = self._tune_cache.pop(sg, None)
                if cfg is not None and self._tune_family.get(self._family(sg)) == cfg:
                    del self._tune_family[self._family(sg)]
                clear[i] = -2
            L.check(L.lib.bsy_plan_set_tuning(h, clear, nops))
            self.tune_stats["invalid_presets"] = self.tune_stats.get("invalid_presets", 0) + len(bad)
        todo = sum(1 for sg in plan.conv_sigs if sg is not None and sg not in self._tune_cache)
        self.tune_stats["autotune_calls"] += 1
        self.tune_stats["timed_ops"] += todo
        self.tune_stats["cached_ops"] += sum(1 for sg in plan.conv_sigs if sg is not None) - todo
        if self.tune_mode == "1":
            L.check(L.lib.bsy_plan_autotune_in_place(h, ext, n, C.c_void_p(stream), 3))
        else:
            L.check(L.lib.bsy_plan_autotune(h, ext, n, C.c_void_p(stream)))
        if todo:
            out = (C.c_int32 * nops)()
            L.check(L.lib.bsy_plan_get_tuning(h, out, nops))
            for sg, c in zip(plan.conv_sigs, out):
                if sg is not None and c >= 0:
                    self._tune_cache.setdefault(sg, int(c))
                    self._tune_family.setdefault(self._family(sg), int(c))
            if self._tune_file:
                try:
                    tmp = self._tune_file + f".{os.getpid()}.tmp"
                    json.dump([[list(k), v] for k, v in self._tune_cache.items()], open(tmp, "w"))
                    os.replace(tmp, self._tune_file)
# ... 218 lines not shown
```

### bs_yolo_amd/lib.py

```python
from __future__ import annotations

import ctypes as C
import os
from pathlib import Path

import torch

PKG = Path(__file__).resolve().parent
LIB_PATH = Path(os.environ["BSY_LIB"]) if os.environ.get("BSY_LIB") else PKG / "libbsyolo_hip.so"

BSY_F16, BSY_F32, BSY_U8 = 0, 1, 2
BSY_EXT_BASE = 0x100000
BSY_MAX_LEVELS = 4
(OP_CONV_FIRST, OP_CONV, OP_DWCONV, OP_SPPF_POOL, OP_ATTN, OP_DECODE, OP_RAW_NCHW, OP_NHWC2NCHW, OP_STEM, OP_BNECK, OP_DWCONV_G, OP_COPY, OP_GAP, OP_MSCA_MIX, OP_MUL, OP_ELA, OP_DWPW, OP_MSCA_SPATIAL, OP_C3K2, OP_S2D, OP_PMSFA_TAIL, OP_CHAIN) = range(22)

SYMBOLS = [
    "bsy_engine_create", "bsy_engine_destroy", "bsy_engine_load_weights", "bsy_plan_create", "bsy_plan_create_arena", "bsy_engine_arena_bytes", "bsy_plan_set_tuning", "bsy_plan_destroy",
    "bsy_plan_run", "bsy_plan_graph_launch", "bsy_plan_profile", "bsy_plan_copy_buffer", "bsy_plan_check_guards", "bsy_plan_autotune", "bsy_plan_get_tuning", "bsy_plan_check_tuning", "bsy_plan_autotune_in_place", "bsy_conv2d", "bsy_conv2d_f32", "bsy_conv2d_f32x", "bsy_conv_first_f32", "bsy_attention_f32", "bsy_conv_packed_dims", "bsy_conv_first", "bsy_stem_fused", "bsy_stem_fused_supported", "bsy_bottleneck_fused", "bsy_bottleneck_fused_supported", "bsy_c3k2_fused", "bsy_c3k2_fused_supported", "bsy_dwconv", "bsy_dwpw_fused", "bsy_dwpw_fused_supported", "bsy_ela", "bsy_ela_scratch_bytes", "bsy_dwconv3x3",
    "bsy_sppf_pool", "bsy_attention", "bsy_detect_decode", "bsy_nms_workspace_bytes", "bsy_nms", "bsy_scale_boxes",
    "bsy_letterbox", "bsy_process_mask", "bsy_process_mask_native", "bsy_scale_masks", "bsy_val_match", "bsy_pack_masks", "bsy_val_match_masks_workspace_bytes", "bsy_val_match_masks", "bsy_val_match_rotated", "bsy_slice_tiles", "bsy_sahi_merge_workspace_bytes",
    "bsy_sahi_merge", "bsy_scale_img", "bsy_tta_merge", "bsy_nms_rotated_workspace_bytes", "bsy_nms_rotated", "bsy_obb_scale", "bsy_end2end_topk_workspace_bytes", "bsy_end2end_topk", "bsy_ap_workspace_bytes", "bsy_ap_per_class", "bsy_last_error", "bsy_version", "bsy_sizeof_op",
]


class View(C.Structure):
    _fields_ = [("buf", C.c_int32), ("ld", C.c_int32), ("coff", C.c_int32), ("C", C.c_int32)]


NO_VIEW = (-1, 0, 0, 0)


class Op(C.Structure):
    _fields_ = [
        ("kind", C.c_int32),
        ("B", C.c_int32), ("H", C.c_int32), ("W", C.c_int32),
        ("OH", C.c_int32), ("OW", C.c_int32),
        ("src0", View), ("src1", View),
        ("up0", C.c_int32), ("up1", C.c_int32),
        ("dst", View), ("res", View),
        ("ksize", C.c_int32), ("stride", C.c_int32), ("pad", C.c_int32),
        ("act", C.c_int32), ("out_f32", C.c_int32),
        ("dst_scale", C.c_int32), ("dst_dy", C.c_int32), ("dst_dx", C.c_int32),
        ("w_off", C.c_int64), ("b_off", C.c_int64),
        ("heads", C.c_int32), ("key_dim", C.c_int32), ("head_dim", C.c_int32),
        ("scale", C.c_float),
        ("nl", C.c_int32), ("nc", C.c_int32), ("nm", C.c_int32), ("A", C.c_int32),
        ("box", View * BSY_MAX_LEVELS), ("cls", View * BSY_MAX_LEVELS),
        ("lvl_h", C.c_int32 * BSY_MAX_LEVELS), ("lvl_w", C.c_int32 * BSY_MAX_LEVELS),
        ("lvl_stride", C.c_float * BSY_MAX_LEVELS),
        ("reserved2", C.c_int32),
        ("in_dtype", C.c_int32), ("out_dtype", C.c_int32),
        ("level", C.c_int32),
        ("lane", C.c_int32), ("tuned_cfg", C.c_int32), ("join", C.c_int32),
        ("mid_c", C.c_int32),
        ("w2_off", C.c_int64), ("b2_off", C.c_int64),
        ("aux_off", C.c_int64 * 18),
        ("prec", C.c_int32), ("ne", C.c_int32), ("ksplit", C.c_int32), ("reserved1", C.c_int32),
        ("msk", View * BSY_MAX_LEVELS),
    ]


class BsyError(RuntimeError):
    pass


def _load() -> C.CDLL:
    if not LIB_PATH.exists():
        raise ImportError(
            f"{LIB_PATH} is missing: build it with `python -m bs_yolo_amd.build` (hipcc, gfx950). "
            "bs_yolo_amd has no CPU fallback.")
    if not os.environ.get("BSY_LIB") and os.environ.get("BSY_ALLOW_STALE_LIB") != "1":
        from .build import stale_sources
        stale = stale_sources()
        if stale:
            raise ImportError(f"{LIB_PATH} was not built from the current sources ({', '.join(stale)} changed or failed to compile): run "
                              "`python -m bs_yolo_amd.build` (BSY_ALLOW_STALE_LIB=1 loads it anyway)")
    lib = C.CDLL(str(LIB_PATH))
    missing = [s for s in SYMBOLS if not hasattr(lib, s)]
    if missing:
        raise ImportError(f"{LIB_PATH} does not export {missing}; rebuild it")
    if lib.bsy_sizeof_op() != C.sizeof(Op):
        raise ImportError(f"{LIB_PATH}: bsy_op is {lib.bsy_sizeof_op()} bytes in the library, {C.sizeof(Op)} in bs_yolo_amd/lib.py; rebuild it")
    vp, i32, i64, f32 = C.c_void_p, C.c_int, C.c_int64, C.c_float
    lib.bsy_last_error.restype = C.c_char_p
    lib.bsy_engine_create.argtypes = [i32, C.POINTER(vp)]
    lib.bsy_engine_destroy.argtypes = [vp]
    lib.bsy_engine_destroy.restype = None
    lib.bsy_engine_load_weights.argtypes = [vp, vp, C.c_size_t]
    lib.bsy_plan_create.argtypes = [vp, C.POINTER(Op), i32, C.POINTER(i64), i32, C.POINTER(vp)]
    lib.bsy_plan_create_arena.argtypes = [vp, C.POINTER(Op), i32, C.POINTER(i64), C.POINTER(i64), i32, i64, C.POINTER(vp)]
    lib.bsy_engine_arena_bytes.argtypes = [vp]
    lib.bsy_engine_arena_bytes.restype = C.c_size_t
    lib.bsy_plan_set_tuning.argtypes = [vp, C.POINTER(C.c_int32), i32]
    lib.bsy_plan_destroy.argtypes = [vp]
    lib.bsy_plan_destroy.restype = None
    lib.bsy_plan_run.argtypes = [vp, C.POINTER(vp), i32, vp]
    lib.bsy_plan_graph_launch.argtypes = [vp, C.POINTER(vp), i32, vp, C.POINTER(i32)]
    lib.bsy_plan_autotune.argtypes = [vp, C.POINTER(vp), i32, vp]
    lib.bsy_plan_get_tuning.argtypes = [vp, C.POINTER(C.c_int32), i32]
    lib.bsy_plan_check_tuning.argtypes = [vp, C.POINTER(vp), i32, C.POINTER(C.c_int32), i32]
    lib.bsy_plan_autotune_in_place.argtypes = [vp, C.POINTER(vp), i32, vp, i32]
    lib.bsy_plan_copy_buffer.argtypes = [vp, i32, vp, C.c_size_t]
    lib.bsy_plan_check_guards.argtypes = [vp, C.POINTER(C.c_int32), C.POINTER(C.c_int64)]
    lib.bsy_plan_profile.argtypes = [vp, C.POINTER(vp), i32, vp, C.POINTER(f32)]
    lib.bsy_conv2d.argtypes = [vp, i32, i32, i32, i32, i32, vp, vp, vp, i32, i32, i32, i32, i32, vp, i32, i32, vp]
    lib.bsy_conv2d_f32.argtypes = [vp, i32, i32, i32, i32, i32, vp, vp, vp, i32, i32, i32, i32, i32, vp, i32, i32, vp]
    lib.bsy_conv2d_f32x.argtypes = [vp, i32, i32, i32, i32, i32, vp, vp, i32, vp, vp, i32, i32, i32, i32, i32, vp, i32, vp]
    lib.bsy_conv_first_f32.argtypes = [vp, i32, i32, i32, i32, vp, vp, vp, i32, i32, i32, i32, i32, i32, vp]
    lib.bsy_attention_f32.argtypes = [vp, i32, i32, i32, i32, i32, i32, f32, vp, i32, i32, vp]
    lib.bsy_conv_packed_dims.argtypes = [i32, i32, i32, C.POINTER(i32), C.POINTER(i32)]
    lib.bsy_conv_first.argtypes = [vp, i32, i32, i32, i32, vp, vp, vp, i32, i32, i32, i32, i32, vp]
    lib.bsy_stem_fused.argtypes = [vp, i32, i32, i32, i32, vp, vp, i32, vp, vp, i32, vp, i32, i32, vp]
    lib.bsy_stem_fused_supported.argtypes = [i32, i32, i32, i32]
    lib.bsy_val_match.argtypes = [vp, i32, vp, i32, i32, vp, vp, vp, i32, C.POINTER(C.c_float), i32, vp, vp]
    lib.bsy_pack_masks.argtypes = [vp, i32, i32, i32, i32, vp, vp, vp]
    lib.bsy_val_match_masks_workspace_bytes.argtypes = [i32, i32, i32]
    lib.bsy_val_match_masks_workspace_bytes.restype = C.c_size_t
    lib.bsy_val_match_masks.argtypes = [vp, i32, vp, i32, i32, vp, vp, vp, vp, i32, vp, vp, i32, C.POINTER(C.c_float), i32, vp, vp, vp,
                                        C.c_size_t, vp]
    lib.bsy_val_match_rotated.argtypes = [vp, i32, vp, i32, i32, vp, vp, vp, i32, C.POINTER(C.c_float), i32, vp, vp, vp]
    lib.bsy_bottleneck_fused.argtypes = [vp, i32, i32, i32, i32, i32, i32, vp, vp, vp, vp, vp, i32, i32, vp]
    lib.bsy_bottleneck_fused_supported.argtypes = [i32, i32]
    lib.bsy_c3k2_fused.argtypes = [vp, i32, i32, i32, i32, i32, i32, i32, vp, vp, vp, vp, vp, vp, vp, vp, vp, i32, vp]
    lib.bsy_c3k2_fused_supported.argtypes = [i32, i32, i32]
    lib.bsy_dwconv.argtypes = [vp, i32, i32, i32, i32, i32, i32, i32, i32, vp, i32, vp, vp, i32, i32, vp]
    lib.bsy_ela_scratch_bytes.argtypes = [i32, i32, i32, i32]
    lib.bsy_dwpw_fused.argtypes = [vp, i32, i32, i32, i32, i32, vp, vp, vp, vp, vp, i32, i32, i32, vp]
    lib.bsy_dwpw_fused_supported.argtypes = [i32, i32]
    lib.bsy_ela_scratch_bytes.restype = C.c_size_t
    lib.bsy_ela.argtypes = [vp, i32, i32, i32, i32, i32, i32, vp, vp, vp, vp, C.POINTER(C.c_float), vp, vp, i32, vp]
    lib.bsy_dwconv3x3.argtypes = [vp, i32, i32, i32, i32, i32, vp, vp, vp, i32, i32, vp, i32, vp]
    lib.bsy_sppf_pool.argtypes = [vp, i32, i32, i32, i32, i32, vp]
    lib.bsy_attention.argtypes = [vp, i32, i32, i32, i32, i32, i32, f32, vp, i32, vp]
    lib.bsy_detect_decode.argtypes = [C.POINTER(vp), C.POINTER(i32), C.POINTER(vp), C.POINTER(i32), C.POINTER(vp),
                                      C.POINTER(i32), C.POINTER(i32), C.POINTER(i32), C.POINTER(f32), i32, i32, i32,
                                      i32, vp, i32, vp]
    lib.bsy_nms_workspace_bytes.argtypes = [i32, i32, i32, i32, i32]
    lib.bsy_nms_workspace_bytes.restype = C.c_size_t
    lib.bsy_nms.argtypes = [vp, i32, i32, i32, i32, i32, f32, f32, vp, i32, i32, i32, i32, i32, f32, i32, vp, vp, vp,
                            C.c_size_t, vp]
    lib.bsy_scale_boxes.argtypes = [vp, vp, i32, i32, i32, vp, vp, vp, vp, vp, vp]
    lib.bsy_nms_rotated_workspace_bytes.argtypes = [i32, i32, i32, i32, i32]
    lib.bsy_nms_rotated_workspace_bytes.restype = C.c_size_t
    lib.bsy_nms_rotated.argtypes = [vp, i32, i32, i32, i32, i32, f32, f32, vp, i32, i32, i32, i32, i32, f32, vp, vp, vp,
                                    C.c_size_t, vp]
    lib.bsy_obb_scale.argtypes = [vp, vp, i32, i32, i32, vp, vp, vp, vp, vp, vp]
    lib.bsy_end2end_topk_workspace_bytes.argtypes = [i32, i32, i32, i32]
    lib.bsy_end2end_topk_workspace_bytes.restype = C.c_size_t
    lib.bsy_end2end_topk.argtypes = [vp, i32, i32, i32, i32, i32, vp, vp, C.c_size_t, vp]
    lib.bsy_process_mask.argtypes = [vp, i32, i32, i32, i32, vp, i32, vp, i32, i32, i32, i32, i32, vp, vp, i32, vp]
    lib.bsy_process_mask_native.argtypes = [vp, i32, i32, i32, i32, vp, i32, vp, i32, i32, i32, i32, i32, i32, i32, i32, vp, vp, i32, vp]
    lib.bsy_scale_masks.argtypes = [vp, i32, i32, i32, i32, i32, i32, i32, i32, i32, i32, vp, vp]
    lib.bsy_letterbox.argtypes = [vp, vp, vp, i32, i32, i32, vp, i32, vp]
    lib.bsy_slice_tiles.argtypes = [vp, i32, i32, i32, vp, i32, i32, i32, i32, vp, i32, vp]
    lib.bsy_ap_workspace_bytes.argtypes = [i32, i32]
    lib.bsy_ap_workspace_bytes.restype = C.c_size_t
    lib.bsy_ap_per_class.argtypes = [vp, vp, vp, i32, i32, vp, vp, i32, vp, vp, C.c_double, vp, vp, vp, vp, vp, vp, C.c_size_t, vp]
    lib.bsy_sahi_merge_workspace_bytes.argtypes = [i32, i32]
    lib.bsy_sahi_merge_workspace_bytes.restype = C.c_size_t
    lib.bsy_sahi_merge.argtypes = [vp, vp, vp, i32, i32, i32, i32, f32, i32, i32, f32, f32, vp, vp, i32, vp, C.c_size_t, vp]
    lib.bsy_scale_img.argtypes = [vp, i32, i32, i32, i32, i32, i32, i32, i32, i32, i32, vp, vp]
    lib.bsy_tta_merge.argtypes = [C.POINTER(vp), C.POINTER(C.c_int32), C.POINTER(C.c_int32), C.POINTER(C.c_int32), C.POINTER(f32),
                                  C.POINTER(C.c_int32), i32, i32, i32, i32, i32, i32, vp, vp]
    return lib


lib = _load()


def check(rc: int) -> None:
    if rc != 0:
        raise BsyError(f"libbsyolo_hip: {lib.bsy_last_error().decode(errors='replace')} (status {rc})")


def stream_ptr(device) -> C.c_void_p:
    return C.c_void_p(torch.cuda.current_stream(device).cuda_stream)


def dtype_code(t) -> int:
    import torch
    if t == torch.float16:
        return BSY_F16
    if t == torch.float32:
        return BSY_F32
    if t == torch.uint8:
        return BSY_U8
    raise TypeError(f"unsupported dtype {t}")
```

### bs_yolo_amd/ops.py

```python
from __future__ import annotations

import ctypes as C
from typing import List, Optional, Sequence

import torch

from . import lib as L


def _stream(t: torch.Tensor):
    return L.stream_ptr(t.device)


def _p(t: Optional[torch.Tensor]):
    return C.c_void_p(t.data_ptr()) if t is not None else None


def pack_conv_weight(w: torch.Tensor, b: Optional[torch.Tensor], device) -> tuple:
    cout, cin, k, _ = w.shape
    cp, kp = C.c_int(), C.c_int()
    L.check(L.lib.bsy_conv_packed_dims(cout, cin, k, C.byref(cp), C.byref(kp)))
    w = w.detach().float().cpu()
    if cin == 3:
        w = torch.cat([w, torch.zeros(cout, 1, k, k)], 1)
        cin = 4
    K = k * k * cin
    wp = torch.zeros(cp.value, kp.value, dtype=torch.float16)
    wp[:cout, :K] = w.permute(0, 2, 3, 1).reshape(cout, K).half()
    bp = torch.zeros(cp.value, dtype=torch.float32)
    if b is not None:
        bp[:cout] = b.detach().float().cpu()
    return wp.to(device), bp.to(device)


def conv2d_nhwc(x: torch.Tensor, wp: torch.Tensor, bp: torch.Tensor, cout: int, k: int, s: int = 1, act: bool = True,
                res: Optional[torch.Tensor] = None, out_f32: bool = False, cin: Optional[int] = None,
                out: Optional[torch.Tensor] = None) -> torch.Tensor:
    assert x.dtype == torch.float16 and x.is_contiguous() and x.dim() == 4
    B, H, W, ld = x.shape
    cin = ld if cin is None else cin
    p = k // 2
    OH, OW = (H + 2 * p - k) // s + 1, (W + 2 * p - k) // s + 1
    if out is None:
        ldy = (cout + 3) // 4 * 4 if out_f32 else (cout + 7) // 8 * 8
        out = torch.zeros((B, OH, OW, ldy), dtype=torch.float32 if out_f32 else torch.float16, device=x.device)
    L.check(L.lib.bsy_conv2d(_p(x), ld, B, H, W, cin, _p(wp), _p(bp), _p(out), out.shape[-1], cout, k, s, int(act),
                             _p(res), res.shape[-1] if res is not None else 0, int(out_f32), _stream(x)))
    return out


def conv2d_nhwc_f32(x: torch.Tensor, w: torch.Tensor, b: torch.Tensor, k: int, s: int = 1, act: bool = True,
                    res: Optional[torch.Tensor] = None, cin: Optional[int] = None, impl: int = 0) -> torch.Tensor:
    assert x.dtype == torch.float32 and x.is_contiguous() and x.dim() == 4
    B, H, W, ld = x.shape
    cin = ld if cin is None else cin
    cout = w.shape[0]
    assert tuple(w.shape) == (cout, cin, k, k)
    wk = w.detach().float().permute(2, 3, 1, 0).reshape(k * k * cin, cout).contiguous().to(x.device)
    bk = b.detach().float().contiguous().to(x.device)
    p = k // 2
    OH, OW = (H + 2 * p - k) // s + 1, (W + 2 * p - k) // s + 1
    ldy = (cout + 3) // 4 * 4
    out = torch.zeros((B, OH, OW, ldy), dtype=torch.float32, device=x.device)
    L.check(L.lib.bsy_conv2d_f32(_p(x), ld, B, H, W, cin, _p(wk), _p(bk), _p(out), ldy, cout, k, s, int(act), _p(res),
                                 res.shape[-1] if res is not None else 0, impl, _stream(x)))
    return out


def conv2d_nhwc_f32x(x: torch.Tensor, w: torch.Tensor, b: torch.Tensor, k: int, s: int = 1, act: bool = True,
                     res: Optional[torch.Tensor] = None, cin: Optional[int] = None) -> torch.Tensor:
    from .weights import split_f16_planes
    assert x.dtype == torch.float32 and x.is_contiguous() and x.dim() == 4
    B, H, W, ld = x.shape
    cin = ld if cin is None else cin
    cout = w.shape[0]
    assert tuple(w.shape) == (cout, cin, k, k)
    hi, lo = split_f16_planes(w.detach().float().cpu().permute(0, 2, 3, 1).reshape(cout, k * k * cin))
    hi, lo = hi.contiguous().to(x.device), lo.contiguous().to(x.device)
    bk = b.detach().float().contiguous().to(x.device)
    p = k // 2
    OH, OW = (H + 2 * p - k) // s + 1, (W + 2 * p - k) // s + 1
    ldy = (cout + 3) // 4 * 4
    out = torch.zeros((B, OH, OW, ldy), dtype=torch.float32, device=x.device)
    L.check(L.lib.bsy_conv2d_f32x(_p(x), ld, B, H, W, cin, _p(hi), _p(lo), hi.shape[1], _p(bk), _p(out), ldy, cout, k, s, int(act),
                                  _p(res), res.shape[-1] if res is not None else 0, _stream(x)))
    return out


def conv_first(img: torch.Tensor, w: torch.Tensor, b: torch.Tensor, k: int = 3, s: int = 2, act: bool = True):
    assert img.is_contiguous() and img.shape[1] == 3
    B, _, H, W = img.shape
    cout = w.shape[0]
    wp, bp = pack_conv_weight(w, b, img.device)
    p = k // 2
    OH, OW = (H + 2 * p - k) // s + 1, (W + 2 * p - k) // s + 1
    out = torch.empty((B, OH, OW, cout), dtype=torch.float16, device=img.device)
    L.check(L.lib.bsy_conv_first(_p(img), L.dtype_code(img.dtype), B, H, W, _p(wp), _p(bp), _p(out), cout, cout, k, s,
                                 int(act), _stream(img)))
    return out


def stem_fused(img: torch.Tensor, w0: torch.Tensor, b0: torch.Tensor, w1: torch.Tensor, b1: torch.Tensor,
               act: bool = True) -> torch.Tensor:
    assert img.is_contiguous() and img.shape[1] == 3
    B, _, H, W = img.shape
    c0, c1 = w0.shape[0], w1.shape[0]
    w0p, b0p = pack_conv_weight(w0, b0, img.device)
    w1p, b1p = pack_conv_weight(w1, b1, img.device)
    oh0, ow0 = (H - 1) // 2 + 1, (W - 1) // 2 + 1
    out = torch.empty((B, (oh0 - 1) // 2 + 1, (ow0 - 1) // 2 + 1, c1), dtype=torch.float16, device=img.device)
    L.check(L.lib.bsy_stem_fused(_p(img), L.dtype_code(img.dtype), B, H, W, _p(w0p), _p(b0p), c0, _p(w1p), _p(b1p), c1,
                                 _p(out), c1, int(act), _stream(img)))
    return out


def bottleneck_fused(x: torch.Tensor, w1: torch.Tensor, b1: torch.Tensor, w2: torch.Tensor, b2: torch.Tensor,
                     out: Optional[torch.Tensor] = None) -> torch.Tensor:
    B, H, W, c = x.shape
    assert x.stride(3) == 1 and x.stride(1) == W * x.stride(2) and x.stride(0) == H * W * x.stride(2)
    ch = w1.shape[0]
    w1p, b1p = pack_conv_weight(w1, b1, x.device)
    w2p, b2p = pack_conv_weight(w2, b2, x.device)
    if out is None:
        out = torch.empty((B, H, W, c), dtype=torch.float16, device=x.device)
    assert out.shape == x.shape and out.stride(3) == 1 and out.stride(1) == W * out.stride(2)
    L.check(L.lib.bsy_bottleneck_fused(_p(x), x.stride(2), B, H, W, c, ch, _p(w1p), _p(b1p), _p(w2p), _p(b2p), _p(out),
                                       out.stride(2), 1, _stream(x)))
    return out


def c3k2_fused(x: torch.Tensor, w1, b1, wa, ba, wb, bb, w4, b4, out: Optional[torch.Tensor] = None) -> torch.Tensor:
# ... 150 lines not shown
```

### bs_yolo_amd/plan.py

```python
from __future__ import annotations

import math
import os
from collections import OrderedDict
from dataclasses import dataclass, field
from typing import Dict, List, Optional, Sequence, Tuple, Union

from . import lib as L


def make_divisible(x, d):
    return math.ceil(x / d) * d


@dataclass
class T:
    buf: int
    ld: int
    coff: int
    C: int
    H: int
    W: int
    up: bool = False
    f32: bool = False
    cmap: Optional[Tuple[int, ...]] = None

    def slice(self, c0: int, c: int) -> "T":
        assert 0 <= c0 and c0 + c <= self.C
        cm = None
        if self.cmap is not None:
            before = sum(1 for v in self.cmap[:c0] if v >= 0)
            cm = tuple(v - before if v >= 0 else -1 for v in self.cmap[c0:c0 + c])
            if all(v >= 0 for v in cm):
                cm = None
        return T(self.buf, self.ld, self.coff + c0, c, self.H, self.W, self.up, self.f32, cm)

    @property
    def real(self) -> int:
        return self.C if self.cmap is None else sum(1 for v in self.cmap if v >= 0)

    def padded(self, pieces: Sequence[Tuple[int, int]]) -> "T":
        cm, base = [], 0
        for width, real in pieces:
            cm += [base + i if i < real else -1 for i in range(width)]
            base += real
        assert len(cm) == self.C
        return T(self.buf, self.ld, self.coff, self.C, self.H, self.W, self.up, self.f32, tuple(cm))

    def view(self):
        return (self.buf, self.ld, self.coff, self.C)


@dataclass
class WRec:
    name: str
    kind: str
    cout: int
    cin: int
    k: int
    perm: Optional[List[int]] = None
    tap: Optional[Tuple[int, int]] = None
    kw: Optional[int] = None
    post: Optional[str] = None
    coef: Tuple[float, float, float] = (0.0, 0.0, 0.0)
    real_cout: int = 0
    real_cin: int = 0
    rows: Optional[List[int]] = None
    cols: Optional[List[int]] = None
    w_off: int = -1
    b_off: int = -1


def stem_supported(c0: int, c1: int, H: int, W: int) -> bool:
    return (c0, c1) in ((32, 64), (16, 32)) and W % 4 == 0 and H >= 4 and W >= 4


def msca_spatial_supported(H: int, W: int) -> bool:
    return H > 0 and W > 0 and H * W <= 1890


def attention_supported(kd: int, hd: int) -> bool:
    return 0 < kd <= 64 and kd % 16 == 0 and 0 < hd <= 128 and hd % 32 == 0


def pmsfa_tail_supported(c: int) -> bool:
    return c in (32, 64)


def dwpw_supported(c: int, cout: int) -> bool:
    return c > 0 and c % 32 == 0 and c <= 256 and cout % 8 == 0


def c3k2_supported(cin: int, c: int, c2: int) -> bool:
    return (cin, c, c2) == (64, 32, 128)


def bneck_supported(c: int, ch: int) -> bool:
    return (c, ch) in ((32, 16), (64, 32))


class Plan:

    EXT_IMG, EXT_Y, EXT_RAW0 = 0, 1, 2
    EXT_PROTO = 5
    EXT_RAW3 = 6

    @classmethod
    def ext_raw(cls, level: int) -> int:
        assert 0 <= level < L.BSY_MAX_LEVELS
        return cls.EXT_RAW0 + level if level < 3 else cls.EXT_RAW3 + level - 3

    def __init__(self, cfg: dict, B: int, H: int, W: int, in_dtype: int = L.BSY_F16, out_dtype: int = L.BSY_F16,
                 fuse_stem: Optional[bool] = None, fuse_bneck: Optional[bool] = None, fuse_head: Optional[bool] = None,
                 fuse_dwpw: Optional[bool] = None, merge_c3k: Optional[bool] = None, fuse_msca: Optional[bool] = None,
                 fuse_tail: Optional[bool] = None, precision: str = "fp16", lanes: Optional[bool] = None, latency: bool = False,
                 fuse_pmsfa: Optional[bool] = None):
        self.cfg, self.B, self.H, self.W = cfg, B, H, W
        self.latency = bool(latency) and precision == "fp16"
        if precision not in ("fp16", "fp32", "fp32x"):
            raise ValueError(f"precision must be 'fp16', 'fp32' or 'fp32x', not {precision!r}")
        self.f32_mode = precision in ("fp32", "fp32x")
        self.split_f16 = precision == "fp32x"
        if self.f32_mode:
            fuse_stem = fuse_bneck = fuse_head = fuse_dwpw = merge_c3k = fuse_msca = fuse_tail = fuse_pmsfa = False
        self.in_dtype, self.out_dtype = in_dtype, out_dtype
        self.fuse_stem = (os.environ.get("BSY_FUSE_STEM", "1") != "0") if fuse_stem is None else bool(fuse_stem)
        self.fuse_bneck = (os.environ.get("BSY_FUSE_BNECK", "1") != "0") if fuse_bneck is None else bool(fuse_bneck)
        self.fuse_head = (os.environ.get("BSY_FUSE_HEAD", "1") != "0") if fuse_head is None else bool(fuse_head)
        self.fuse_boxtail = self.fuse_head and os.environ.get("BSY_FUSE_BOXTAIL", "1") != "0"
        self.fuse_dwpw = (os.environ.get("BSY_FUSE_DWPW", "1") != "0") if fuse_dwpw is None else bool(fuse_dwpw)
        self.merge_c3k = (os.environ.get("BSY_MERGE_C3K", "1") != "0") if merge_c3k is None else bool(merge_c3k)
        self.fuse_msca = (os.environ.get("BSY_FUSE_MSCA", "1") != "0") if fuse_msca is None else bool(fuse_msca)
        self.fuse_tail = (os.environ.get("BSY_FUSE_TAIL", "1") != "0") if fuse_tail is None else bool(fuse_tail)
        self.fuse_pmsfa = (os.environ.get("BSY_FUSE_PMSFA", "1") != "0") if fuse_pmsfa is None else bool(fuse_pmsfa)
        self.buf_bytes: List[int] = []
        self.ops: List[dict] = []
        self.wrecs: "OrderedDict[str, WRec]" = OrderedDict()
        self.flops = 0
        self.meta: Dict = {}
        self._lane = 0
        self._build()
        if self.latency:
            self._apply_split_k()
        env = os.environ.get("BSY_LANES")
        if env == "0" or (env is None and not lanes and (lanes is not None or B * H * W < 12 * 640 * 640)):
            for o in self.ops:
                if "lane" in o:
                    o["lane"] = 0
        assert all(o.get("lane", 0) == 0 or o["kind"] in (L.OP_CONV, L.OP_DWCONV, L.OP_BNECK, L.OP_DWCONV_G, L.OP_DWPW, L.OP_C3K2) for o in self.ops)

    @staticmethod
    def split_factors(k: int, stride: int, cin: int, c0: int, cout: int, OH: int, OW: int) -> Tuple[int, int]:
        if cin % 64 or c0 % 64 or cout % 8:
            return 1, 1
        steps = k * k * cin // 64
        tiles = -(-OH * OW // 128) * -(-cout // 128)
        want = min(32 // max(tiles, 1), 8, steps // 4)
        if steps < 32 or want < 3:
            return 1, 1
        nt = 3 if k == 3 else 1
        n64 = cin // 64
        nc = max((d for d in range(1, n64 + 1) if n64 % d == 0 and d * nt <= want), default=1)
        return (nc, nt) if nc * nt >= 3 else (1, 1)

    def _apply_split_k(self) -> None:
        for o in self.ops:
            if o["kind"] != L.OP_CONV or o.get("out_f32", 0) or o.get("dst_scale", 1) != 1 or o["ksize"] not in (1, 3):
                continue
            s0, s1 = o["src0"], o.get("src1")
            cin = s0.C + (s1.C if s1 else 0)
            cout = o.get("cout", o["dst"].C)
            if o["dst"].ld % 8 or (o.get("res") is not None and o["res"].ld % 8):
                continue
            nc, nt = self.split_factors(o["ksize"], o["stride"], cin, s0.C if s1 else cin, cout, o["OH"], o["OW"])
            if nc * nt < 2:
                continue
            ldw = (cout + 31) // 32 * 32
            self.buf_bytes.append(nc * nt * self.B * o["OH"] * o["OW"] * ldw * 4)
            o["box"] = [T(len(self.buf_bytes) - 1, ldw, 0, ldw, o["OH"], o["OW"], False, True)]
            o["ksplit"] = nc | (nt << 8)

    def alloc(self, C: int, H: int, W: int, f32: bool = False) -> T:
        if self.f32_mode:
            self.buf_bytes.append(self.B * H * W * make_divisible(C, 8) * 4)
            return T(len(self.buf_bytes) - 1, make_divisible(C, 8), 0, C, H, W, False, True)
        ld = make_divisible(C, 4) if f32 else make_divisible(C, 8)
        self.buf_bytes.append(self.B * H * W * ld * (4 if f32 else 2))
        return T(len(self.buf_bytes) - 1, ld, 0, C, H, W, False, f32)

    def _wrec(self, key: str, **kw) -> str:
        if key not in self.wrecs:
            self.wrecs[key] = WRec(**kw)
        return key

    def conv(self, name: str, src: Union[T, Sequence[T]], cout: int, k: int = 1, s: int = 1, act: bool = True,
             dst: Optional[T] = None, res: Optional[T] = None, plain: bool = False, out_f32: bool = False,
             perm: Optional[List[int]] = None, name2: Optional[str] = None, wkind: Optional[str] = None,
             wshape: Optional[Tuple[int, int, int]] = None, real: Tuple[int, int] = (0, 0),
             rows: Optional[List[int]] = None, cols: Optional[List[int]] = None) -> T:
        srcs = [src] if isinstance(src, T) else list(src)
        assert 1 <= len(srcs) <= 2, "at most two concat operands per conv"
        H, W = srcs[0].H, srcs[0].W
        assert all(t.H == H and t.W == W and (t.f32 == self.f32_mode) for t in srcs)
        cin = sum(t.C for t in srcs)
        if not self.f32_mode and any(t.C % 8 or t.coff % 8 for t in srcs):
            raise NotImplementedError(f"{name}: source channels / offsets {[(t.C, t.coff) for t in srcs]} are not multiples of 8 (fp16 path)")
        p = k // 2
        OH, OW = (H + 2 * p - k) // s + 1, (W + 2 * p - k) // s + 1
        if dst is None:
            dst = self.alloc(cout, OH, OW, out_f32)
        assert dst.C == cout and dst.H == OH and dst.W == OW and dst.f32 == (out_f32 or self.f32_mode) and not dst.up
        if res is not None:
            assert res.C == cout and res.H == OH and res.W == OW and not res.up
        if rows is None and cols is None and (any(t.cmap is not None for t in srcs) or dst.cmap is not None):
            assert perm is None and wshape is None and not real[1]
            out_real = real[0] or dst.real
            rows = list(dst.cmap) if dst.cmap is not None else [i if i < out_real else -1 for i in range(cout)]
            cols, base = [], 0
            for t in srcs:
                cols += [base + v if v >= 0 else -1 for v in (t.cmap if t.cmap is not None else range(t.C))]
                base += t.real
            real = (out_real, base)
            if real[0] < cout and dst.cmap is None:
                dst = dst.padded([(cout, real[0])])
        if name2 is not None:
            assert not plain and perm is None and cout % 2 == 0
            key = self._wrec(name + "+" + name2, name=name, kind="conv2", cout=cout, cin=cin, k=k, post=name2, rows=rows, cols=cols,
                             real_cout=real[0], real_cin=real[1])
        else:
            wc, wi, wk = wshape or (cout, cin, k)
            key = self._wrec(name, name=name, kind=wkind or ("plain" if plain else "conv"), cout=wc, cin=wi, k=wk, perm=perm,
                             real_cout=real[0], real_cin=real[1], rows=rows, cols=cols)
        self.ops.append(dict(kind=L.OP_CONV, H=H, W=W, OH=OH, OW=OW, src0=srcs[0],
                             src1=srcs[1] if len(srcs) > 1 else None, dst=dst, res=res, ksize=k, stride=s, pad=p,
                             act=int(act), out_f32=int(out_f32), wkey=key, dst_scale=1, name=name, lane=self._lane, cout=cout,
                             mfma_flops=2 * self.B * OH * OW * cout * cin * k * k))
        self.flops += 2 * self.B * OH * OW * cout * cin * k * k
        return dst

    def conv_first(self, name: str, cout: int, k: int, s: int, p: Optional[int] = None) -> T:
        p = k // 2 if p is None else p
        if (k, s, p) == (6, 2, 2) and not self.f32_mode:
            assert self.H % 2 == 0 and self.W % 2 == 0
            sd = self.alloc(16, self.H // 2, self.W // 2)
            self.ops.append(dict(kind=L.OP_S2D, H=self.H, W=self.W, OH=self.H // 2, OW=self.W // 2,
                                 src0=T(L.BSY_EXT_BASE + self.EXT_IMG, 0, 0, 3, self.H, self.W), dst=sd, in_dtype=self.in_dtype,
                                 name=name + ".s2d"))
            return self.conv(name, sd, cout, 3, 1, wkind="first_s2d", wshape=(cout, 3, 6))
        OH, OW = (self.H + 2 * p - k) // s + 1, (self.W + 2 * p - k) // s + 1
        dst = self.alloc(cout, OH, OW)
# ... 435 lines not shown
                    assert isinstance(x, T)
                    k = args[1] if len(args) > 1 else 1
                    s = args[2] if len(args) > 2 else 1
                    if c2 != x.C:
                        raise NotImplementedError(f"DWConv {x.C} -> {c2}: only the depthwise case c1 == c2 is accelerated")
                    y = self.dwconv_g(name, x, k, k, s, x.C)
                elif m == "C3k2":
                    legacy = False
                    c3k = bool(args[1]) if len(args) > 1 else False
                    e = args[2] if len(args) > 2 else 0.5
                    if scale and scale in "mlx":
                        c3k = True
                    y = self.c2f(name, x, c2, n, True, e, "c3k" if c3k else "bottleneck")
                elif m == "C3k2_gai":
                    c3k = bool(args[1]) if len(args) > 1 else False
                    e = args[2] if len(args) > 2 else 0.5
                    y = self.c2f(name, x, c2, n, True, e, "c3k_gai" if c3k else "pmsfa")
                elif m == "SCDown":
                    assert isinstance(x, T)
                    y = self.scdown(name, x, c2, args[1], args[2])
                elif m == "C2f":
                    shortcut = bool(args[1]) if len(args) > 1 else False
                    y = self.c2f(name, x, c2, n, shortcut, 0.5, "c2f")
                elif m == "C2":
                    shortcut = bool(args[1]) if len(args) > 1 else True
                    y = self.c2(name, x, c2, n, shortcut)
                elif m == "SPPF":
                    assert isinstance(x, T) and (len(args) < 2 or args[1] == 5)
                    y = self.sppf(name, x, c2)
                else:
                    assert isinstance(x, T)
                    y = self.c2psa(name, x, c2, n)
                cout = c2
            elif m == "MSCAAttention":
                assert isinstance(x, T)
                y = self.msca(name, x)
                cout = x.C
            elif m == "ELA":
                assert isinstance(x, T)
                y = self.ela(name, x)
                cout = x.C
            elif m == "nn.Upsample":
                assert isinstance(x, T) and not x.up and args[1] == 2 and args[2] == "nearest"
                y = T(x.buf, x.ld, x.coff, x.C, x.H * 2, x.W * 2, True, x.f32)
                cout = x.C
            elif m == "Concat":
                assert isinstance(x, list) and len(x) == 2, "only two-operand Concat feeding a conv is accelerated"
                for j, t in enumerate(x):
                    if isinstance(t, list):
                        assert all(isinstance(u, T) for u in t)
                        real = self.alloc(sum(u.C for u in t), t[0].H, t[0].W)
                        c0 = 0
                        for u in t:
                            self.copy(f"{name}.cat{j}", u, real.slice(c0, u.C))
                            c0 += u.C
                        x[j] = real
                assert all(isinstance(t, T) for t in x)
                y = list(x)
                cout = sum(t.C for t in x)
            elif m in ("Detect", "Segment", "OBB"):
                xs = x if isinstance(x, list) else [x]
                assert all(isinstance(t, T) for t in xs)
                if m == "Segment":
                    nm = args[1]
                    npr = make_divisible(min(args[2], max_ch) * width, 8)
                    self.proto(name + ".proto", xs[0], npr, nm)
                    self.detect(name, xs, args[0], legacy, nm=nm)
                elif m == "OBB":
                    ne = args[1] if len(args) > 1 and not isinstance(args[1], (list, tuple)) else 1
                    if ne != 1:
                        raise NotImplementedError(f"OBB with ne = {ne}: dist2rbox (utils/tal.py:404-423) decodes one angle")
                    self.detect(name, xs, args[0], legacy, ne=ne)
                else:
                    self.detect(name, xs, args[0], legacy)
                y, cout = None, 0
            else:
                raise NotImplementedError(f"module {m} is not on the accelerated path")
            outs.append(y)
            chans.append(cout)
            x = y
        self.layer_out = outs
        self.meta.update(scale=scale, n_layers=len(layers), legacy=legacy)
        self._fuse_stem()

    def _fuse_stem(self):
        if not self.fuse_stem or len(self.ops) < 2:
            return
        a, b = self.ops[0], self.ops[1]
        if a["kind"] != L.OP_CONV_FIRST or b["kind"] != L.OP_CONV:
            return
        mid = a["dst"]
        if (b["src0"] is not mid or b.get("src1") is not None or b.get("res") is not None or b["ksize"] != 3
                or b["stride"] != 2 or b["out_f32"] or not b["act"] or a["ksize"] != 3 or a["stride"] != 2):
            return
        if not stem_supported(mid.C, b["dst"].C, self.H, self.W):
            return
        for o in self.ops[2:]:
            for key in ("src0", "src1", "res"):
                t = o.get(key)
                if t is not None and t.buf == mid.buf:
                    return
        self.buf_bytes[mid.buf] = 16
        self.ops[0:2] = [dict(kind=L.OP_STEM, H=self.H, W=self.W, OH=b["OH"], OW=b["OW"], src0=a["src0"], dst=b["dst"],
                              ksize=3, stride=2, pad=1, act=1, wkey=a["wkey"], wkey2=b["wkey"], mid_c=mid.C,
                              in_dtype=self.in_dtype, name=a["name"] + "+" + b["name"].split(".")[-1], lane=0,
                              mfma_flops=a["mfma_flops"] + b["mfma_flops"])]
        self.layer_out[0] = None

    _VIEW_KEYS = ("src0", "src1", "dst", "res")
    _LIST_KEYS = ("box", "cls", "msk")

    def op_buffers(self, o: dict) -> List[int]:
        out = []
        for k in self._VIEW_KEYS:
            t = o.get(k)
            if t is not None and t.buf < L.BSY_EXT_BASE:
                out.append(t.buf)
        for k in self._LIST_KEYS:
            for t in o.get(k, []) or []:
                if t is not None and t.buf < L.BSY_EXT_BASE:
                    out.append(t.buf)
        return out

    def buffer_lifetimes(self) -> List[Optional[Tuple[int, int]]]:
        n = len(self.ops)
        life: List[Optional[List[int]]] = [None] * len(self.buf_bytes)
        for i, o in enumerate(self.ops):
            for b in self.op_buffers(o):
                if life[b] is None:
                    life[b] = [i, i]
                else:
                    life[b][1] = i
        i = 0
        while i < n:
            if self.ops[i].get("lane", 0) > 0:
                start = i
                end = n - 1
                for j in range(i + 1, n):
                    if self.ops[j].get("join", 0):
                        end = j
                        break
                for j in range(start, end + 1):
                    if self.ops[j].get("lane", 0) > 0:
                        for b in self.op_buffers(self.ops[j]):
                            life[b][0] = min(life[b][0], start)
                            life[b][1] = max(life[b][1], end)
                i = end + 1
            else:
                i += 1
        return [tuple(x) if x is not None else None for x in life]

    def assign_offsets(self, reuse: bool = True) -> Tuple[List[int], int]:
        sizes = [(b + 255) & ~255 for b in self.buf_bytes]
        offs = [0] * len(sizes)
        if not reuse:
            off = 0
            for i, sz in enumerate(sizes):
                offs[i] = off
                off += sz
            return offs, off
        life = self.buffer_lifetimes()
        placed: List[int] = []
        top = 0
        for i in sorted(range(len(sizes)), key=lambda k: (-sizes[k], k)):
            if life[i] is None or sizes[i] == 0:
                continue
            busy = sorted((offs[j], offs[j] + sizes[j]) for j in placed
                          if not (life[j][1] < life[i][0] or life[i][1] < life[j][0]))
            at = 0
            for lo, hi in busy:
                if at + sizes[i] <= lo:
                    break
                at = max(at, hi)
            offs[i] = at
            placed.append(i)
            top = max(top, at + sizes[i])
        return offs, top

    def conv_signature(self, o: dict) -> Optional[tuple]:
        if o["kind"] != L.OP_CONV or self.f32_mode:
            return None
        s0, s1, d, r = o["src0"], o.get("src1"), o["dst"], o.get("res")
        return (self.B, o["H"], o["W"], s0.C, s0.ld, int(s0.up), s1.C if s1 else 0, s1.ld if s1 else 0, int(s1.up) if s1 else 0,
                o.get("cout", d.C), d.ld, o["ksize"], o["stride"], int(r is not None), r.ld if r is not None else 0,
                o.get("out_f32", 0), o.get("dst_scale", 1), o.get("act", 0), o.get("ksplit", 0))

    def c_ops(self):
        arr = (L.Op * len(self.ops))()
        for o, d in zip(arr, self.ops):
            def v(t):
                return L.View(*(t.view() if t is not None else L.NO_VIEW))
            o.kind = d["kind"]
            o.B, o.H, o.W, o.OH, o.OW = self.B, d["H"], d["W"], d["OH"], d["OW"]
            o.src0, o.src1 = v(d.get("src0")), v(d.get("src1"))
            o.up0 = int(bool(d.get("src0") and d["src0"].up))
            o.up1 = int(bool(d.get("src1") and d["src1"].up))
            o.dst, o.res = v(d.get("dst")), v(d.get("res"))
            o.ksize, o.stride, o.pad = d.get("ksize", 0), d.get("stride", 0), d.get("pad", 0)
            o.act, o.out_f32 = d.get("act", 0), d.get("out_f32", 0)
            o.dst_scale, o.dst_dy, o.dst_dx = d.get("dst_scale", 1), d.get("dst_dy", 0), d.get("dst_dx", 0)
            if "wkey" in d:
                w = self.wrecs[d["wkey"]]
                assert w.w_off >= 0, "pack weights before serialising"
                o.w_off, o.b_off = w.w_off, w.b_off
            if "wkey2" in d:
                w = self.wrecs[d["wkey2"]]
                assert w.w_off >= 0, "pack weights before serialising"
                o.w2_off, o.b2_off = w.w_off, w.b_off
            o.mid_c = d.get("mid_c", 0)
            for j, k in enumerate(d.get("wkeys", [])):
                w = self.wrecs[k]
                assert w.w_off >= 0, "pack weights before serialising"
                o.aux_off[2 * j], o.aux_off[2 * j + 1] = w.w_off, w.b_off
            if d["kind"] == L.OP_ELA:
                cf = self.wrecs[d["wkey"]].coef
                d = dict(d, scale=cf[0], lvl_stride=[cf[1], cf[2]])
            o.heads, o.key_dim, o.head_dim, o.scale = d.get("heads", 0), d.get("key_dim", 0), d.get("head_dim", 0), \
                d.get("scale", 0.0)
            o.nl, o.nc, o.nm, o.A = d.get("nl", 0), d.get("nc", 0), d.get("nm", 0), d.get("A", 0)
            o.ne = d.get("ne", 0)
            for j in range(L.BSY_MAX_LEVELS):
                o.box[j] = v(d["box"][j] if j < len(d.get("box", [])) else None)
                o.cls[j] = v(d["cls"][j] if j < len(d.get("cls", [])) else None)
                o.msk[j] = v(d["msk"][j] if j < len(d.get("msk", [])) else None)
                o.lvl_h[j] = d["lvl_h"][j] if j < len(d.get("lvl_h", [])) else 0
                o.lvl_w[j] = d["lvl_w"][j] if j < len(d.get("lvl_w", [])) else 0
                o.lvl_stride[j] = d["lvl_stride"][j] if j < len(d.get("lvl_stride", [])) else 0.0
            o.in_dtype, o.out_dtype, o.level = d.get("in_dtype", 0), d.get("out_dtype", 0), d.get("level", 0)
            o.lane, o.join, o.tuned_cfg = d.get("lane", 0), d.get("join", 0), 0
            o.prec = (2 if self.split_f16 else 1) if self.f32_mode else 0
            o.ksplit = d.get("ksplit", 0)
        return arr
```

### include/bsyolo.h

```cpp
#ifndef BSYOLO_H
#define BSYOLO_H

#include <stddef.h>
#include <stdint.h>

#ifdef __cplusplus
extern "C" {
#endif

typedef void* bsy_stream;

enum bsy_status {
    BSY_OK = 0,
    BSY_ERR_ARG = -1,
    BSY_ERR_HIP = -2,
    BSY_ERR_ALLOC = -3,
    BSY_ERR_STATE = -4
};

enum bsy_dtype { BSY_F16 = 0, BSY_F32 = 1, BSY_U8 = 2 };

typedef struct bsy_engine bsy_engine;
typedef struct bsy_plan bsy_plan;

// ... 6 lines not shown
enum bsy_op_kind {
    BSY_OP_CONV_FIRST = 0,
    BSY_OP_CONV = 1,
    BSY_OP_DWCONV = 2,
    BSY_OP_SPPF_POOL = 3,
    BSY_OP_ATTN = 4,
    BSY_OP_DECODE = 5,
    BSY_OP_RAW_NCHW = 6,
    BSY_OP_NHWC2NCHW = 7,
    BSY_OP_STEM = 8,
    BSY_OP_BNECK = 9,
    BSY_OP_DWCONV_G = 10,
    BSY_OP_COPY = 11,
    BSY_OP_GAP = 12,
    BSY_OP_MSCA_MIX = 13,
    BSY_OP_MUL = 14,
    BSY_OP_DWPW = 16,
    BSY_OP_MSCA_SPATIAL = 17,
    BSY_OP_C3K2 = 18,
    BSY_OP_S2D = 19,
    BSY_OP_PMSFA_TAIL = 20,
    BSY_OP_ELA = 15
};

typedef struct bsy_op {
    int32_t kind;
    int32_t B, H, W;
    int32_t OH, OW;
    bsy_view src0, src1;
    int32_t up0, up1;
    bsy_view dst;
    bsy_view res;
    int32_t ksize, stride, pad;
    int32_t act;
    int32_t out_f32;
    int32_t dst_scale, dst_dy, dst_dx;
    int64_t w_off, b_off;
    int32_t heads, key_dim, head_dim;
    float scale;
    int32_t nl, nc, nm, A;
    bsy_view box[BSY_MAX_LEVELS], cls[BSY_MAX_LEVELS];
    int32_t lvl_h[BSY_MAX_LEVELS], lvl_w[BSY_MAX_LEVELS];
    float lvl_stride[BSY_MAX_LEVELS];
    int32_t reserved2;
    int32_t in_dtype, out_dtype;
    int32_t level;
    int32_t lane;
    int32_t tuned_cfg;
    int32_t join;
    int32_t mid_c;
    int64_t w2_off, b2_off;
    int64_t aux_off[18];
    int32_t prec;
    int32_t ne;
    int32_t ksplit;
    int32_t reserved1;
    bsy_view msk[BSY_MAX_LEVELS];
} bsy_op;

int bsy_sizeof_op(void);
int bsy_engine_create(int device, bsy_engine** out);
void bsy_engine_destroy(bsy_engine* e);
int bsy_engine_load_weights(bsy_engine* e, const void* host_blob, size_t bytes);

int bsy_plan_create(bsy_engine* e, const bsy_op* ops, int n_ops, const int64_t* buf_bytes, int n_bufs, bsy_plan** out);
int bsy_plan_create_arena(bsy_engine* e, const bsy_op* ops, int n_ops, const int64_t* buf_bytes, const int64_t* buf_off, int n_bufs,
                          int64_t arena_bytes, bsy_plan** out);
size_t bsy_engine_arena_bytes(const bsy_engine* e);
void bsy_plan_destroy(bsy_plan* p);
int bsy_plan_run(bsy_plan* p, void* const* ext, int n_ext, bsy_stream stream);
int bsy_plan_graph_launch(bsy_plan* p, void* const* ext, int n_ext, bsy_stream stream, int* captured);
int bsy_plan_autotune(bsy_plan* p, void* const* ext, int n_ext, bsy_stream stream);
int bsy_plan_set_tuning(bsy_plan* p, const int32_t* cfg, int n_ops);
int bsy_plan_get_tuning(bsy_plan* p, int32_t* out, int n_ops);
int bsy_plan_check_tuning(bsy_plan* p, void* const* ext, int n_ext, int32_t* valid, int n_ops);
int bsy_plan_autotune_in_place(bsy_plan* p, void* const* ext, int n_ext, bsy_stream stream, int rounds);
int bsy_plan_check_guards(bsy_plan* p, int32_t* bad_buf, int64_t* bad_off);
int bsy_plan_copy_buffer(bsy_plan* p, int buf, void* host_dst, size_t bytes);
int bsy_plan_profile(bsy_plan* p, void* const* ext, int n_ext, bsy_stream stream, float* ms_per_op );


int bsy_conv2d(const void* x, int ldx, int B, int H, int W, int C1, const void* w, const float* b, void* y, int ldy,
               int C2, int ksize, int stride, int act, const void* res, int ldr, int y_f32, bsy_stream stream);
int bsy_conv2d_f32(const float* x, int ldx, int B, int H, int W, int C1, const float* w, const float* b, float* y, int ldy,
                   int C2, int ksize, int stride, int act, const float* res, int ldr, int impl, bsy_stream stream);
int bsy_conv2d_f32x(const float* x, int ldx, int B, int H, int W, int C1, const void* w_hi, const void* w_lo, int k_pad,
                    const float* b, float* y, int ldy, int C2, int ksize, int stride, int act, const float* res, int ldr,
                    bsy_stream stream);
int bsy_conv_first_f32(const void* img, int img_dtype, int B, int H, int W, const float* w, const float* b, float* y, int ldy,
                       int C2, int ksize, int stride, int act, int impl, bsy_stream stream);
int bsy_attention_f32(const float* qkv, int ld, int B, int N, int heads, int key_dim, int head_dim, float scale, float* out,
                      int ldo, int impl, bsy_stream stream);
int bsy_conv_packed_dims(int C2, int C1, int ksize, int* cout_pad, int* k_pad);

int bsy_conv_first(const void* img, int img_dtype, int B, int H, int W, const void* w, const float* b, void* y,
                   int ldy, int C2, int ksize, int stride, int act, bsy_stream stream);

int bsy_stem_fused(const void* img, int img_dtype, int B, int H, int W, const void* w0, const float* b0, int C0,
                   const void* w1, const float* b1, int C1, void* y, int ldy, int act, bsy_stream stream);
int bsy_stem_fused_supported(int C0, int C1, int H, int W);

int bsy_bottleneck_fused(const void* x, int ldx, int B, int H, int W, int C, int CH, const void* w1, const float* b1,
                         const void* w2, const float* b2, void* y, int ldy, int act, bsy_stream stream);
int bsy_bottleneck_fused_supported(int C, int CH);
int bsy_c3k2_fused(const void* x, int ldx, int B, int H, int W, int Cin, int c, int C2, const void* w1, const float* b1, const void* wa,
                   const float* ba, const void* wb, const float* bb, const void* w4, const float* b4, void* y, int ldy, bsy_stream stream);
int bsy_c3k2_fused_supported(int Cin, int c, int C2);

int bsy_dwconv(const void* x, int ldx, int B, int H, int W, int C, int kh, int kw, int stride, const float* w, int wld,
               const float* b, void* y, int ldy, int act, bsy_stream stream);
size_t bsy_ela_scratch_bytes(int B, int H, int W, int C);
int bsy_ela(const void* x, int ldx, int B, int H, int W, int C, int k, const float* wsp, const float* wch,
            const float* gnw, const float* gnb, const float* coef, void* scratch, void* y, int ldy, bsy_stream stream);

int bsy_dwpw_fused(const void* x, int ldx, int B, int H, int W, int C, const float* dww, const float* dwb, const void* w,
                   const float* b, void* y, int ldy, int C2, int act, bsy_stream stream);
int bsy_dwpw_fused_supported(int C, int C2);

int bsy_dwconv3x3(const void* x, int ldx, int B, int H, int W, int C, const float* w, const float* b, void* y, int ldy,
                  int act, const void* res, int ldr, bsy_stream stream);

int bsy_sppf_pool(void* buf, int ld, int B, int H, int W, int C, bsy_stream stream);

int bsy_attention(const void* qkv, int ld, int B, int N, int heads, int key_dim, int head_dim, float scale, void* out,
                  int ldo, bsy_stream stream);

int bsy_detect_decode(const float* const* box, const int* ldb, const float* const* cls, const int* ldc,
                      const float* const* msk, const int* ldm, const int* lvl_h, const int* lvl_w,
                      const float* lvl_stride, int nl, int B, int nc, int nm, void* y, int y_dtype, bsy_stream stream);

size_t bsy_nms_workspace_bytes(int B, int A, int nc, int multi_label, int max_nms);
int bsy_nms(void* pred, int pred_dtype, int B, int nc, int nm, int A, float conf_thres, float iou_thres,
            const int32_t* classes, int n_classes, int agnostic, int multi_label, int max_det, int max_nms,
            float max_wh, int in_place, float* out, int32_t* counts, void* workspace, size_t workspace_bytes,
            bsy_stream stream);

size_t bsy_nms_rotated_workspace_bytes(int B, int A, int nc, int multi_label, int max_nms);
int bsy_nms_rotated(void* pred, int pred_dtype, int B, int nc, int ne, int A, float conf_thres, float iou_thres,
                    const int32_t* classes, int n_classes, int agnostic, int multi_label, int max_det, int max_nms,
                    float max_wh, float* out, int32_t* counts, void* workspace, size_t workspace_bytes, bsy_stream stream);
int bsy_obb_scale(float* det, const int32_t* counts, int B, int max_det, int row, const float* gain, const float* pad_x,
                  const float* pad_y, const float* h0, const float* w0, bsy_stream stream);

size_t bsy_end2end_topk_workspace_bytes(int B, int A, int nc, int max_det);
int bsy_end2end_topk(const void* pred, int pred_dtype, int B, int nc, int A, int max_det, float* out, void* workspace,
                     size_t workspace_bytes, bsy_stream stream);

int bsy_scale_boxes(float* det, const int32_t* counts, int B, int max_det, int row, const float* gain,
                    const float* pad_x, const float* pad_y, const float* h0, const float* w0, bsy_stream stream);

int bsy_letterbox(const uint8_t* const* imgs, const int32_t* hw, const int32_t* geom, int B, int H2, int W2, void* out,
                  int out_dtype, bsy_stream stream);

int bsy_process_mask(const void* protos, int proto_dtype, int nm, int mh, int mw, const float* coef, int ldc,
                     const float* boxes, int ldb, int n, int ih, int iw, int upsample, float* lowres, void* out,
                     int out_dtype, bsy_stream stream);

int bsy_process_mask_native(const void* protos, int proto_dtype, int nm, int mh, int mw, const float* coef, int ldc,
                            const float* boxes, int ldb, int n, int top, int left, int bottom, int right, int oh, int ow,
                            float* lowres, void* out, int out_dtype, bsy_stream stream);
int bsy_scale_masks(const void* masks, int dtype, int n, int mh, int mw, int top, int left, int bottom, int right, int oh, int ow,
                    void* out, bsy_stream stream);

int bsy_val_match(const float* det, int row, const int32_t* counts, int B, int max_det, const float* gt_boxes,
                  const float* gt_cls, const int32_t* gt_counts, int Lmax, const float* iouv, int n_iou,
                  unsigned char* out, bsy_stream stream);
// ... 39 lines not shown
```

Before: 21000.

## Fuse following 1x1 conv into 3x3 conv GEMM epilogue via LDS tile

Adds a TAIL1 variant of the MFMA conv kernel. After the 3x3 conv it parks the activated tile in LDS and multiplies it by streamed 1x1 weights, so the 3x3-then-1x1 pair becomes one launch. The planner fuses eligible pairs above a pixel threshold, and the intermediate activation never goes to global memory. In exchange the kernel needs more LDS and holds the full Cout in one tile (ntn=1), which may cut parallelism and occupancy on some layers.

Measured after the change: 21050, median of 2. About the same (+0.2%).

```diff
diff --git a/bs_yolo_amd/csrc/common.h b/bs_yolo_amd/csrc/common.h
--- a/bs_yolo_amd/csrc/common.h
+++ b/bs_yolo_amd/csrc/common.h
@@ -56,6 +56,7 @@
     const float* tail_bias;
     int nsl_c = 0, nsl_t = 0;
     float* split_ws = nullptr;
+    int tail1_cout = 0, tail1_act = 0;
 };
 int launch_conv(const ConvArgs& a, hipStream_t s);
 #define BSY_CONV_MAX_CFG 64
diff --git a/bs_yolo_amd/csrc/conv_gemm.hip b/bs_yolo_amd/csrc/conv_gemm.hip
--- a/bs_yolo_amd/csrc/conv_gemm.hip
+++ b/bs_yolo_amd/csrc/conv_gemm.hip
@@ -3,7 +3,7 @@
 
 __device__ __attribute__((aligned(16))) unsigned int bsy_zero_page[16];
 
-template <int KS, int WAVES_M, int WAVES_N, int MT, int NT, int STAGES, bool ALIGNED, int BK>
+template <int KS, int WAVES_M, int WAVES_N, int MT, int NT, int STAGES, bool ALIGNED, int BK, bool TAIL1 = false>
 __global__ __launch_bounds__(64 * WAVES_M * WAVES_N) void conv_mfma_kernel(const ConvK p) {
     constexpr int NW = WAVES_M * WAVES_N;
     constexpr int NTHR = 64 * NW;
@@ -20,7 +20,14 @@
     constexpr int NDMA = PIW + WIW;
     constexpr int SWS = BK == 32 ? 2 : 1;
     constexpr int OTILE = (TM > TN ? TM : TN) * ((TM > TN ? TN : TM) + 8);
-    constexpr int SMEM = STAGES * STAGE > OTILE ? STAGES * STAGE : OTILE;
+    static_assert(!TAIL1 || (KS == 3 && ALIGNED && STAGES == 2), "the 1x1 tail stage: aligned 3x3 tiles with a two-stage ring");
+    constexpr int T1_CH = NW * 512;
+    constexpr int T1_KC = T1_CH / TN;
+    constexpr int T1_NBUF = !TAIL1 ? 0 : TN == 256 ? 3 : TN / T1_KC;
+    constexpr bool T1_EARLY = TAIL1 && OTILE >= STAGES * STAGE;
+    constexpr int SMEM0 = STAGES * STAGE > OTILE ? STAGES * STAGE : OTILE;
+    constexpr int SMEM = SMEM0 > OTILE + T1_NBUF * T1_CH ? SMEM0 : OTILE + T1_NBUF * T1_CH;
+    static_assert(SMEM * 2 <= 160 * 1024, "LDS budget");
     __shared__ __attribute__((aligned(16))) half_t smem[SMEM];
 
     const int tid = threadIdx.x;
@@ -173,12 +180,22 @@
     for (int a = 0; a < NT; ++a)
 #pragma unroll
         for (int b = 0; b < MT; ++b) {
-            acc_bias(acc[a][b], p.bias + n0 + (wn * NT + a) * 32, lh);
+            acc_bias(acc[a][b], p.bias + (TAIL1 ? min((wn * NT + a) * 32, ((p.Cout + 127) & ~127) - 32) : n0 + (wn * NT + a) * 32), lh);
             if (slice) {
 #pragma unroll
                 for (int r = 0; r < 16; ++r) acc[a][b][r] = 0.f;
             }
         }
+
+    const int t1_nkc = TAIL1 ? p.Cout / T1_KC : 0;
+    const bsy_rsrc_t rst = make_rsrc(TAIL1 ? p.tail_wgt : p.wgt, TAIL1 ? (unsigned)(((p.tail1_cout + 127) & ~127) * p.Cout * 2) : 0u);
+    const unsigned t1_voff = 2u * (unsigned)((wave * 32 % TN + (lane >> 1)) * p.Cout + (wave * 32 / TN) * 16 + (((lane & 1) ^ ((lane >> 4) & 1)) << 3));
+    int t1_issued = 0;
+    auto t1_issue = [&](const int c, const int buf) {
+        dma16_buf(rst, t1_voff, 2u * (unsigned)(c * T1_KC), smem + OTILE + buf * T1_CH + wave * 512);
+    };
+    if (T1_EARLY)
+        for (; t1_issued < T1_NBUF && t1_issued < t1_nkc; ++t1_issued) t1_issue(t1_issued, t1_issued);
 
 #pragma unroll
     for (int s = 0; s < STAGES - 1; ++s)
@@ -231,6 +248,53 @@
         return;
     }
 #endif
+    if constexpr (TAIL1) {
+        __syncthreads();
+        if (!T1_EARLY)
+            for (; t1_issued < T1_NBUF && t1_issued < t1_nkc; ++t1_issued) t1_issue(t1_issued, t1_issued);
+        tile_park<TN, MT, NT>(p.act, acc, smem, wm, wn, lrow, lh);
+#pragma unroll
+        for (int a = 0; a < NT; ++a)
+#pragma unroll
+            for (int b = 0; b < MT; ++b) acc_bias(acc[a][b], p.tail_bias + min((wn * NT + a) * 32, ((p.tail1_cout + 127) & ~127) - 32), lh);
+        constexpr int LDT = TN + 8;
+        int buf = 0;
+        for (int kc = 0; kc < t1_nkc; ++kc) {
+            switch (t1_issued - 1 - kc) {
+                case 0: asm volatile("s_waitcnt vmcnt(0) lgkmcnt(0)" ::: "memory"); break;
+                case 1: asm volatile("s_waitcnt vmcnt(1) lgkmcnt(0)" ::: "memory"); break;
+                case 2: asm volatile("s_waitcnt vmcnt(2) lgkmcnt(0)" ::: "memory"); break;
+                case 3: asm volatile("s_waitcnt vmcnt(3) lgkmcnt(0)" ::: "memory"); break;
+                case 4: asm volatile("s_waitcnt vmcnt(4) lgkmcnt(0)" ::: "memory"); break;
+                case 5: asm volatile("s_waitcnt vmcnt(5) lgkmcnt(0)" ::: "memory"); break;
+                case 6: asm volatile("s_waitcnt vmcnt(6) lgkmcnt(0)" ::: "memory"); break;
+                default: asm volatile("s_waitcnt vmcnt(7) lgkmcnt(0)" ::: "memory"); break;
+            }
+            __builtin_amdgcn_s_barrier();
+            if (kc > 0 && t1_issued < t1_nkc) { t1_issue(t1_issued, buf ? buf - 1 : T1_NBUF - 1); ++t1_issued; }
+            const half_t* sT = smem + OTILE + buf * T1_CH;
+#pragma unroll
+            for (int ks = 0; ks < T1_KC / 16; ++ks) {
+                half8 bfr[MT], afr[NT];
+#pragma unroll
+                for (int b = 0; b < MT; ++b)
+                    bfr[b] = *reinterpret_cast<const half8*>(smem + ((wm * MT + b) * 32 + lrow) * LDT + kc * T1_KC + 16 * ks + 8 * lh);
+#pragma unroll
+                for (int a = 0; a < NT; ++a)
+                    afr[a] = *reinterpret_cast<const half8*>(sT + (ks * TN + (wn * NT + a) * 32 + lrow) * 16 + ((lh ^ ((lrow >> 3) & 1)) << 3));
+#pragma unroll
+                for (int a = 0; a < NT; ++a)
+#pragma unroll
+                    for (int b = 0; b < MT; ++b) acc[a][b] = __builtin_amdgcn_mfma_f32_32x32x16_f16(afr[a], bfr[b], acc[a][b], 0, 0, 0);
+            }
+            if (++buf == T1_NBUF) buf = 0;
+        }
+        __syncthreads();
+        tile_park<TN, MT, NT>(p.tail1_act, acc, smem, wm, wn, lrow, lh);
+        __syncthreads();
+        tile_store<TM, TN, NTHR>(smem, reinterpret_cast<half_t*>(p.dst), p.ldd, m0, p.M, p.tail1_cout, tid);
+        return;
+    }
     if (split) {
         float* ws = p.split_ws + (size_t)slice * (size_t)p.slab;
 #pragma unroll
@@ -318,6 +382,30 @@
         HIP_TRY(hipGetLastError());
     }
     return BSY_OK;
+}
+
+template <int WM, int WN, int MT, int NT, int BK>
+static int launch_tail1(const ConvK& k, hipStream_t s) {
+    constexpr int TM = WM * MT * 32;
+    ConvK p = k;
+    p.ntn = 1;
+    const long long nblk = ceil_div(k.M, TM);
+    if (nblk <= 0 || nblk > 0x7fffffffLL) BSY_FAIL(BSY_ERR_ARG, "conv: grid %lld out of range", nblk);
+    hipLaunchKernelGGL((conv_mfma_kernel<3, WM, WN, MT, NT, 2, true, BK, true>), dim3((unsigned)nblk), dim3(64 * WM * WN), 0, s, p);
+    HIP_TRY(hipGetLastError());
+    return BSY_OK;
+}
+
+int launch_tail1_cfg(int id, const ConvK& k, hipStream_t s) {
+    switch (id) {
+        case 0x22: return launch_tail1<2, 2, 2, 2, 32>(k, s);
+        case 0x23: return launch_tail1<2, 2, 2, 2, 64>(k, s);
+        case 0x42: return launch_tail1<4, 2, 2, 2, 32>(k, s);
+        case 0x43: return launch_tail1<4, 2, 2, 2, 64>(k, s);
+        case 0x72: return launch_tail1<4, 2, 2, 4, 32>(k, s);
+        case 0x73: return launch_tail1<4, 2, 2, 4, 64>(k, s);
+    }
+    BSY_FAIL(BSY_ERR_ARG, "conv: no 1x1-tail kernel is built for configuration 0x%02x", id);
 }
 
 template <int WM, int WN, int MT, int NT, int S, bool AL, int BK>
diff --git a/bs_yolo_amd/csrc/conv_kernels.h b/bs_yolo_amd/csrc/conv_kernels.h
--- a/bs_yolo_amd/csrc/conv_kernels.h
+++ b/bs_yolo_amd/csrc/conv_kernels.h
@@ -33,6 +33,7 @@
     float* split_ws;
     long long slab;
     int korder;
+    int tail1_cout, tail1_act;
 };
 
 __device__ __forceinline__ void dma16(const void* g, half_t* lds_wave_base) {
@@ -337,8 +338,46 @@
     }
 }
 
+template <int TN, int MT, int NT>
+__device__ __forceinline__ void tile_park(int act, f32x16 (&acc)[NT][MT], half_t* stile, int wm, int wn, int lrow, int lh) {
+    constexpr int LDT = TN + 8;
+#pragma unroll
+    for (int b = 0; b < MT; ++b) {
+        const int prow = (wm * MT + b) * 32 + lrow;
+#pragma unroll
+        for (int a = 0; a < NT; ++a) {
+            const int cl = (wn * NT + a) * 32;
+#pragma unroll
+            for (int g = 0; g < 4; ++g) {
+                const int c = cl + 8 * g + 4 * lh;
+                half4 o;
+                f32x4 t = f32x4{acc[a][b][4 * g], acc[a][b][4 * g + 1], acc[a][b][4 * g + 2], acc[a][b][4 * g + 3]};
+                if (act) t = silu4_f(t);
+#pragma unroll
+                for (int e = 0; e < 4; ++e) o[e] = (half_t)t[e];
+                *reinterpret_cast<half4*>(stile + prow * LDT + c) = o;
+            }
+        }
+    }
+}
+template <int TM, int TN, int NTHR>
+__device__ __forceinline__ void tile_store(const half_t* stile, half_t* dst, int ldd, int m0, int M, int C, int tid) {
+    constexpr int LDT = TN + 8;
+    constexpr int CPRW = TN / 8;
+    constexpr int ITER = TM * CPRW / NTHR;
+#pragma unroll
+    for (int i = 0; i < ITER; ++i) {
+        const int id = tid + NTHR * i;
+        const int row = id / CPRW, cc = (id % CPRW) * 8;
+        const int m = m0 + row;
+        if (m >= M || cc >= C) continue;
+        *reinterpret_cast<half8*>(dst + (size_t)m * ldd + cc) = *reinterpret_cast<const half8*>(stile + row * LDT + cc);
+    }
+}
+
 int launch_gemm_cfg(int id, int ksize, const ConvK& k, hipStream_t s);
 int launch_stream1x1_cfg(int id, const ConvK& k, hipStream_t s);
 int launch_patch_cfg(int id, bool tail, const ConvK& k, hipStream_t s);
+int launch_tail1_cfg(int id, const ConvK& k, hipStream_t s);
 
 constexpr int PERSIST_MAX_COUT = 1024;
diff --git a/bs_yolo_amd/csrc/conv_select.hip b/bs_yolo_amd/csrc/conv_select.hip
--- a/bs_yolo_amd/csrc/conv_select.hip
+++ b/bs_yolo_amd/csrc/conv_select.hip
@@ -16,7 +16,7 @@
     return (a.stride == 2 && !(Cin & 63) && !(a.C0 & 63)) ? 2 : 1;
 }
 
-enum ConvFam { CONV_GEMM, CONV_PERSIST, CONV_WRES, CONV_PATCH, CONV_TAIL };
+enum ConvFam { CONV_GEMM, CONV_PERSIST, CONV_WRES, CONV_PATCH, CONV_TAIL, CONV_GEMM_TAIL1 };
 struct ConvCfg {
     int id; ConvFam fam;
     int tm, tn, stages, bk;
@@ -25,6 +25,9 @@
 };
 template <int WM, int WN, int MT, int NT, int S, bool AL, int BK> constexpr ConvCfg gemm_row(int id) {
     return {id, CONV_GEMM, WM * MT * 32, WN * NT * 32, S, BK, AL, 0, 0};
+}
+template <int WM, int WN, int MT, int NT, int BK> constexpr ConvCfg tail1_row(int id) {
+    return {id, CONV_GEMM_TAIL1, WM * MT * 32, WN * NT * 32, 2, BK, true, 0, 0};
 }
 template <int WM, int WN, int MT, int NT, int S, int BK> constexpr ConvCfg persist_row(int id) {
     return {id, CONV_PERSIST, WM * MT * 32, WN * NT * 32, S, BK, true, 0, 0};
@@ -90,19 +93,33 @@
     wres_row<2, 3, 24>(0xE2),
     wres_row<1, 4, 32>(0xF1),
     wres_row<1, 3, 32>(0xF2),
+    tail1_row<2, 2, 2, 2, 32>(0x22),
+    tail1_row<2, 2, 2, 2, 64>(0x23),
+    tail1_row<4, 2, 2, 2, 32>(0x42),
+    tail1_row<4, 2, 2, 2, 64>(0x43),
+    tail1_row<4, 2, 2, 4, 32>(0x72),
+    tail1_row<4, 2, 2, 4, 64>(0x73),
 };
 
-static const ConvCfg* conv_cfg_row(int cfg, bool tail) {
-    for (const ConvCfg& r : kConvCfgs) if (r.id == (cfg & ~4) && (r.fam == CONV_TAIL) == tail) return &r;
+static int conv_form(const ConvArgs& a) { return !a.tail_wgt ? 0 : a.epi ? 1 : 2; }
+static const ConvCfg* conv_cfg_row(int cfg, int form) {
+    for (const ConvCfg& r : kConvCfgs)
+        if (r.id == (cfg & ~4) && (r.fam == CONV_TAIL ? 1 : r.fam == CONV_GEMM_TAIL1 ? 2 : 0) == form) return &r;
     return nullptr;
 }
 
 bool conv_cfg_valid(const ConvArgs& a, int cfg) {
-    const ConvCfg* r = conv_cfg_row(cfg, a.tail_wgt != nullptr);
+    const ConvCfg* r = conv_cfg_row(cfg, conv_form(a));
     if (!r) return false;
     const int Cin = a.C0 + a.C1, ko = conv_korder(a), nsl = a.nsl_c * a.nsl_t;
     const bool aligned = !(Cin & 31) && !(a.C0 & 31), aligned64 = !(Cin & 63) && !(a.C0 & 63);
     if ((r->aligned && !aligned) || (r->bk == 64 && !aligned64)) return false;
+    if (r->fam == CONV_GEMM_TAIL1) {
+        if (!(cfg & 4) != !ko || !ko || (ko == 1 && r->bk == 64)) return false;
+        if (a.ksize != 3 || a.C1 || a.up0 || a.res || nsl > 1 || a.epi || a.out_f32 || a.dst_scale > 1) return false;
+        if ((a.ldd & 7) || ((uintptr_t)a.dst & 15) || !a.tail_bias || ((uintptr_t)a.tail_wgt & 15) || ((uintptr_t)a.tail_bias & 15)) return false;
+        return aligned64 && a.Cout > 0 && a.Cout <= r->tn && !(a.Cout & 31) && a.tail1_cout > 0 && a.tail1_cout <= r->tn && !(a.tail1_cout & 7);
+    }
     if (r->fam == CONV_GEMM) {
         if (!(cfg & 4) != !ko) return false;
         if (ko && (!r->aligned || (ko == 1 && r->bk == 64))) return false;
@@ -135,6 +152,13 @@
         for (int i = 0; i < n; ++i) if (out[i] == c) return;
         if (n < max_out && conv_cfg_valid(a, c)) out[n++] = c;
     };
+    if (a.tail_wgt && !a.epi) {
+        const bool wide = a.Cout > 128 || a.tail1_cout > 128;
+        const int v = ko == 2 ? 3 : 2;
+        add((wide ? 0x70 : 0x20) | v | km);
+        for (const ConvCfg& r : kConvCfgs) if (r.fam == CONV_GEMM_TAIL1) add(r.id | km);
+        return n;
+    }
     if (a.tail_wgt) {
         if (t20) { add(0xD2); add(0xD1); add(0xD3); }
         add(0xB2); add(0xB1); add(0xB3); add(0xD2); add(0xD1); add(0xD3);
@@ -202,8 +226,7 @@
     k.res = a.res; k.ldr = a.ldr; k.act = a.act; k.B = a.B; k.tiles_x = k.tiles_y = 0;
     k.epi = a.epi; k.y = a.y; k.y_f32 = a.y_f32; k.A = a.A; k.a0 = a.a0; k.nrows = a.nrows; k.lvl_stride = a.lvl_stride;
     k.raw = a.raw; k.raw_f32 = a.raw_f32; k.rawC = a.rawC;
-    k.tail_wgt = a.tail_wgt; k.tail_bias = a.tail_bias;
-    if (a.tail_wgt && !a.epi) BSY_FAIL(BSY_ERR_ARG, "conv: a box-branch tail needs the decoder arguments (epi 3)");
+    k.tail_wgt = a.tail_wgt; k.tail_bias = a.tail_bias; k.tail1_cout = a.tail1_cout; k.tail1_act = a.tail1_act;
     k.dst_scale = a.dst_scale > 0 ? a.dst_scale : 1; k.dst_dy = a.dst_dy; k.dst_dx = a.dst_dx; k.ntn = 1;
     k.nsl_c = k.nsl_t = 1; k.cb_per = Cin; k.taps_per = a.ksize * a.ksize; k.split_ws = nullptr; k.slab = 0; k.ldw = 0;
     if (a.nsl_c * a.nsl_t > 1) {
@@ -232,9 +255,10 @@
         cfg = list[0];
     }
     k.korder = conv_korder(a);
-    const ConvCfg* r = conv_cfg_row(cfg, a.tail_wgt != nullptr);
+    const ConvCfg* r = conv_cfg_row(cfg, conv_form(a));
     switch (r->fam) {
         case CONV_GEMM: return launch_gemm_cfg(r->id, a.ksize, k, s);
+        case CONV_GEMM_TAIL1: return launch_tail1_cfg(r->id, k, s);
         case CONV_PERSIST:
         case CONV_WRES: return launch_stream1x1_cfg(r->id, k, s);
         case CONV_PATCH:
diff --git a/bs_yolo_amd/csrc/engine.hip b/bs_yolo_amd/csrc/engine.hip
--- a/bs_yolo_amd/csrc/engine.hip
+++ b/bs_yolo_amd/csrc/engine.hip
@@ -522,6 +522,11 @@
                     a.Cout = op.mid_c;
                     a.tail_wgt = (const half_t*)(wb + op.w2_off); a.tail_bias = (const float*)(wb + op.b2_off);
                 }
+            }
+            if (op.out_f32 == 0 && op.mid_c > 0) {
+                a.Cout = op.mid_c; a.act = op.act & 1;
+                a.tail1_cout = op.dst.C; a.tail1_act = (op.act >> 1) & 1;
+                a.tail_wgt = (const half_t*)(wb + op.w2_off); a.tail_bias = (const float*)(wb + op.b2_off);
             }
             if (op.ksplit > 0 && op.out_f32 == 0) {
                 a.nsl_c = op.ksplit & 255; a.nsl_t = (op.ksplit >> 8) & 255;
@@ -866,6 +871,38 @@
     return launch_conv(a, (hipStream_t)stream);
 }
 
+static void tail1_args(ConvArgs& a, const void* x, int ldx, int B, int H, int W, int C1, const void* w, const float* b, int C2, int stride, int act,
+                       const void* w2, const float* b2, int C3, int act2, void* y, int ldy, const void* res, int ldr) {
+    memset(&a, 0, sizeof(a));
+    a.src0 = (const half_t*)x; a.ld0 = ldx; a.C0 = C1; a.B = B; a.H = H; a.W = W;
+    a.ksize = 3; a.stride = stride; a.pad = 1;
+    a.OH = stride > 0 ? (H + 2 - 3) / stride + 1 : 0; a.OW = stride > 0 ? (W + 2 - 3) / stride + 1 : 0;
+    a.wgt = (const half_t*)w; a.bias = b; a.dst = y; a.ldd = ldy; a.Cout = C2; a.act = act; a.dst_scale = 1;
+    a.res = (const half_t*)res; a.ldr = ldr;
+    a.tail_wgt = (const half_t*)w2; a.tail_bias = b2; a.tail1_cout = C3; a.tail1_act = act2;
+    a.cfg = -1;
+}
+
+extern "C" int bsy_conv2d_tail1(const void* x, int ldx, int B, int H, int W, int C1, const void* w, const float* b, int C2, int stride, int act,
+                                const void* w2, const float* b2, int C3, int act2, void* y, int ldy, const void* res, int ldr, int cfg,
+                                bsy_stream stream) {
+    if (!x || !w || !b || !w2 || !b2 || !y) BSY_FAIL(BSY_ERR_ARG, "conv2d_tail1: null pointer");
+    ConvArgs a;
+    tail1_args(a, x, ldx, B, H, W, C1, w, b, C2, stride, act, w2, b2, C3, act2, y, ldy, res, ldr);
+    a.cfg = cfg;
+    if (a.cfg >= 0 && !conv_cfg_valid(a, a.cfg)) BSY_FAIL(BSY_ERR_ARG, "conv2d_tail1: configuration 0x%02x is not valid for this shape", a.cfg);
+    return launch_conv(a, (hipStream_t)stream);
+}
+
+extern "C" int bsy_conv2d_tail1_configs(const void* x, int ldx, int B, int H, int W, int C1, const void* w, const float* b, int C2, int stride,
+                                        int act, const void* w2, const float* b2, int C3, int act2, void* y, int ldy, const void* res, int ldr,
+                                        int* out, int max_out) {
+    if (!x || !w || !b || !w2 || !b2 || !y || !out || max_out <= 0) return 0;
+    ConvArgs a;
+    tail1_args(a, x, ldx, B, H, W, C1, w, b, C2, stride, act, w2, b2, C3, act2, y, ldy, res, ldr);
+    return conv_candidates(a, out, max_out);
+}
+
 extern "C" int bsy_conv2d_f32(const float* x, int ldx, int B, int H, int W, int C1, const float* w, const float* b, float* y, int ldy,
                               int C2, int ksize, int stride, int act, const float* res, int ldr, int impl, bsy_stream stream) {
     if (!x || !w || !b || !y) BSY_FAIL(BSY_ERR_ARG, "conv2d_f32: null pointer");
diff --git a/bs_yolo_amd/engine.py b/bs_yolo_amd/engine.py
--- a/bs_yolo_amd/engine.py
+++ b/bs_yolo_amd/engine.py
@@ -22,7 +22,8 @@
                  fuse_bneck: Optional[bool] = None, fuse_head: Optional[bool] = None, fuse_dwpw: Optional[bool] = None,
                  merge_c3k: Optional[bool] = None, fuse_msca: Optional[bool] = None, fuse_tail: Optional[bool] = None,
                  max_plans: Optional[int] = None, precision: str = "fp16", graph: Optional[bool] = None, graph_ring: int = 3,
-                 latency: Optional[bool] = None, fuse_pmsfa: Optional[bool] = None):
+                 latency: Optional[bool] = None, fuse_pmsfa: Optional[bool] = None, fuse_cv1: Optional[bool] = None,
+                 tail1_min_pixels: Optional[int] = None):
         if not torch.cuda.is_available():
             raise RuntimeError("bs_yolo_amd needs a ROCm GPU (there is no CPU fallback)")
         self.cfg = cfg
@@ -68,6 +69,8 @@
         self.fuse_msca = fuse_msca
         self.fuse_tail = fuse_tail
         self.fuse_pmsfa = fuse_pmsfa
+        self.fuse_cv1 = fuse_cv1
+        self.tail1_min_pixels = tail1_min_pixels
         self._packed = Plan(cfg, 1, 64, 64, **self._fuse_kw())
         blob = pack_plan_weights(self._packed, state_dict, bn_eps)
         self.weight_bytes = len(blob)
@@ -94,7 +97,7 @@
         return dict(fuse_stem=self.fuse_stem, fuse_bneck=self.fuse_bneck, fuse_head=self.fuse_head, fuse_dwpw=self.fuse_dwpw,
                     merge_c3k=self.merge_c3k, fuse_msca=self.fuse_msca, fuse_tail=self.fuse_tail, precision=self.precision,
                     lanes=True if getattr(self, "graph", False) else None, latency=getattr(self, "latency", False),
-                    fuse_pmsfa=self.fuse_pmsfa)
+                    fuse_pmsfa=self.fuse_pmsfa, fuse_cv1=self.fuse_cv1, tail1_min_pixels=self.tail1_min_pixels)
 
     def plan_for(self, B: int, H: int, W: int, in_dtype: torch.dtype, out_dtype: torch.dtype):
         key = (B, H, W, in_dtype, out_dtype)
diff --git a/bs_yolo_amd/lib.py b/bs_yolo_amd/lib.py
--- a/bs_yolo_amd/lib.py
+++ b/bs_yolo_amd/lib.py
@@ -16,7 +16,7 @@
 
 SYMBOLS = [
     "bsy_engine_create", "bsy_engine_destroy", "bsy_engine_load_weights", "bsy_plan_create", "bsy_plan_create_arena", "bsy_engine_arena_bytes", "bsy_plan_set_tuning", "bsy_plan_destroy",
-    "bsy_plan_run", "bsy_plan_graph_launch", "bsy_plan_profile", "bsy_plan_copy_buffer", "bsy_plan_check_guards", "bsy_plan_autotune", "bsy_plan_get_tuning", "bsy_plan_check_tuning", "bsy_plan_autotune_in_place", "bsy_conv2d", "bsy_conv2d_f32", "bsy_conv2d_f32x", "bsy_conv_first_f32", "bsy_attention_f32", "bsy_conv_packed_dims", "bsy_conv_first", "bsy_stem_fused", "bsy_stem_fused_supported", "bsy_bottleneck_fused", "bsy_bottleneck_fused_supported", "bsy_c3k2_fused", "bsy_c3k2_fused_supported", "bsy_dwconv", "bsy_dwpw_fused", "bsy_dwpw_fused_supported", "bsy_ela", "bsy_ela_scratch_bytes", "bsy_dwconv3x3",
+    "bsy_plan_run", "bsy_plan_graph_launch", "bsy_plan_profile", "bsy_plan_copy_buffer", "bsy_plan_check_guards", "bsy_plan_autotune", "bsy_plan_get_tuning", "bsy_plan_check_tuning", "bsy_plan_autotune_in_place", "bsy_conv2d", "bsy_conv2d_tail1", "bsy_conv2d_tail1_configs", "bsy_conv2d_f32", "bsy_conv2d_f32x", "bsy_conv_first_f32", "bsy_attention_f32", "bsy_conv_packed_dims", "bsy_conv_first", "bsy_stem_fused", "bsy_stem_fused_supported", "bsy_bottleneck_fused", "bsy_bottleneck_fused_supported", "bsy_c3k2_fused", "bsy_c3k2_fused_supported", "bsy_dwconv", "bsy_dwpw_fused", "bsy_dwpw_fused_supported", "bsy_ela", "bsy_ela_scratch_bytes", "bsy_dwconv3x3",
     "bsy_sppf_pool", "bsy_attention", "bsy_detect_decode", "bsy_nms_workspace_bytes", "bsy_nms", "bsy_scale_boxes",
     "bsy_letterbox", "bsy_process_mask", "bsy_process_mask_native", "bsy_scale_masks", "bsy_val_match", "bsy_pack_masks", "bsy_val_match_masks_workspace_bytes", "bsy_val_match_masks", "bsy_val_match_rotated", "bsy_slice_tiles", "bsy_sahi_merge_workspace_bytes",
     "bsy_sahi_merge", "bsy_scale_img", "bsy_tta_merge", "bsy_nms_rotated_workspace_bytes", "bsy_nms_rotated", "bsy_obb_scale", "bsy_end2end_topk_workspace_bytes", "bsy_end2end_topk", "bsy_ap_workspace_bytes", "bsy_ap_per_class", "bsy_last_error", "bsy_version", "bsy_sizeof_op",
@@ -104,6 +104,9 @@
     lib.bsy_plan_check_guards.argtypes = [vp, C.POINTER(C.c_int32), C.POINTER(C.c_int64)]
     lib.bsy_plan_profile.argtypes = [vp, C.POINTER(vp), i32, vp, C.POINTER(f32)]
     lib.bsy_conv2d.argtypes = [vp, i32, i32, i32, i32, i32, vp, vp, vp, i32, i32, i32, i32, i32, vp, i32, i32, vp]
+    lib.bsy_conv2d_tail1.argtypes = [vp, i32, i32, i32, i32, i32, vp, vp, i32, i32, i32, vp, vp, i32, i32, vp, i32, vp, i32, i32, vp]
+    lib.bsy_conv2d_tail1_configs.argtypes = [vp, i32, i32, i32, i32, i32, vp, vp, i32, i32, i32, vp, vp, i32, i32, vp, i32, vp, i32,
+                                             C.POINTER(C.c_int32), i32]
     lib.bsy_conv2d_f32.argtypes = [vp, i32, i32, i32, i32, i32, vp, vp, vp, i32, i32, i32, i32, i32, vp, i32, i32, vp]
     lib.bsy_conv2d_f32x.argtypes = [vp, i32, i32, i32, i32, i32, vp, vp, i32, vp, vp, i32, i32, i32, i32, i32, vp, i32, vp]
     lib.bsy_conv_first_f32.argtypes = [vp, i32, i32, i32, i32, vp, vp, vp, i32, i32, i32, i32, i32, i32, vp]
diff --git a/bs_yolo_amd/ops.py b/bs_yolo_amd/ops.py
--- a/bs_yolo_amd/ops.py
+++ b/bs_yolo_amd/ops.py
@@ -47,6 +47,26 @@
     L.check(L.lib.bsy_conv2d(_p(x), ld, B, H, W, cin, _p(wp), _p(bp), _p(out), out.shape[-1], cout, k, s, int(act),
                              _p(res), res.shape[-1] if res is not None else 0, int(out_f32), _stream(x)))
     return out
+
+
+def _tail1_args(x, wp, bp, c2, s, act, wp2, bp2, c3, act2, out, res, cin):
+    assert x.dtype == torch.float16 and x.is_contiguous() and x.dim() == 4 and out.dtype == torch.float16
+    B, H, W, ld = x.shape
+    return (_p(x), ld, B, H, W, ld if cin is None else cin, _p(wp), _p(bp), c2, s, int(act), _p(wp2), _p(bp2), c3, int(act2), _p(out),
+            out.shape[-1], _p(res), res.shape[-1] if res is not None else 0)
+
+
+def conv2d_tail1_nhwc(x: torch.Tensor, wp: torch.Tensor, bp: torch.Tensor, c2: int, s: int, act: bool, wp2: torch.Tensor,
+                      bp2: torch.Tensor, c3: int, act2: bool, out: torch.Tensor, res: Optional[torch.Tensor] = None,
+                      cin: Optional[int] = None, cfg: int = -1) -> torch.Tensor:
+    L.check(L.lib.bsy_conv2d_tail1(*_tail1_args(x, wp, bp, c2, s, act, wp2, bp2, c3, act2, out, res, cin), cfg, _stream(x)))
+    return out
+
+
+def conv2d_tail1_configs(x, wp, bp, c2, s, act, wp2, bp2, c3, act2, out, res=None, cin=None) -> List[int]:
+    ids = (C.c_int32 * 64)()
+    n = L.lib.bsy_conv2d_tail1_configs(*_tail1_args(x, wp, bp, c2, s, act, wp2, bp2, c3, act2, out, res, cin), ids, 64)
+    return [int(ids[i]) for i in range(n)]
 
 
 def conv2d_nhwc_f32(x: torch.Tensor, w: torch.Tensor, b: torch.Tensor, k: int, s: int = 1, act: bool = True,
diff --git a/bs_yolo_amd/plan.py b/bs_yolo_amd/plan.py
--- a/bs_yolo_amd/plan.py
+++ b/bs_yolo_amd/plan.py
@@ -7,6 +7,9 @@
 from typing import Dict, List, Optional, Sequence, Tuple, Union
 
 from . import lib as L
+
+
+TAIL1_MIN_PIXELS = 51200
 
 
 def make_divisible(x, d):
@@ -114,7 +117,7 @@
                  fuse_stem: Optional[bool] = None, fuse_bneck: Optional[bool] = None, fuse_head: Optional[bool] = None,
                  fuse_dwpw: Optional[bool] = None, merge_c3k: Optional[bool] = None, fuse_msca: Optional[bool] = None,
                  fuse_tail: Optional[bool] = None, precision: str = "fp16", lanes: Optional[bool] = None, latency: bool = False,
-                 fuse_pmsfa: Optional[bool] = None):
+                 fuse_pmsfa: Optional[bool] = None, fuse_cv1: Optional[bool] = None, tail1_min_pixels: Optional[int] = None):
         self.cfg, self.B, self.H, self.W = cfg, B, H, W
         self.latency = bool(latency) and precision == "fp16"
         if precision not in ("fp16", "fp32", "fp32x"):
@@ -122,7 +125,7 @@
         self.f32_mode = precision in ("fp32", "fp32x")
         self.split_f16 = precision == "fp32x"
         if self.f32_mode:
-            fuse_stem = fuse_bneck = fuse_head = fuse_dwpw = merge_c3k = fuse_msca = fuse_tail = fuse_pmsfa = False
+            fuse_stem = fuse_bneck = fuse_head = fuse_dwpw = merge_c3k = fuse_msca = fuse_tail = fuse_pmsfa = fuse_cv1 = False
         self.in_dtype, self.out_dtype = in_dtype, out_dtype
         self.fuse_stem = (os.environ.get("BSY_FUSE_STEM", "1") != "0") if fuse_stem is None else bool(fuse_stem)
         self.fuse_bneck = (os.environ.get("BSY_FUSE_BNECK", "1") != "0") if fuse_bneck is None else bool(fuse_bneck)
@@ -133,6 +136,8 @@
         self.fuse_msca = (os.environ.get("BSY_FUSE_MSCA", "1") != "0") if fuse_msca is None else bool(fuse_msca)
         self.fuse_tail = (os.environ.get("BSY_FUSE_TAIL", "1") != "0") if fuse_tail is None else bool(fuse_tail)
         self.fuse_pmsfa = (os.environ.get("BSY_FUSE_PMSFA", "1") != "0") if fuse_pmsfa is None else bool(fuse_pmsfa)
+        self.fuse_cv1 = (os.environ.get("BSY_FUSE_CV1", "1") != "0") if fuse_cv1 is None else bool(fuse_cv1)
+        self.tail1_min_pixels = int(os.environ.get("BSY_CV1_MIN_PIXELS", TAIL1_MIN_PIXELS)) if tail1_min_pixels is None else int(tail1_min_pixels)
         self.buf_bytes: List[int] = []
         self.ops: List[dict] = []
         self.wrecs: "OrderedDict[str, WRec]" = OrderedDict()
@@ -165,7 +170,7 @@
 
     def _apply_split_k(self) -> None:
         for o in self.ops:
-            if o["kind"] != L.OP_CONV or o.get("out_f32", 0) or o.get("dst_scale", 1) != 1 or o["ksize"] not in (1, 3):
+            if o["kind"] != L.OP_CONV or o.get("out_f32", 0) or o.get("dst_scale", 1) != 1 or o["ksize"] not in (1, 3) or o.get("tail1_c"):
                 continue
             s0, s1 = o["src0"], o.get("src1")
             cin = s0.C + (s1.C if s1 else 0)
@@ -767,6 +772,7 @@
         self.layer_out = outs
         self.meta.update(scale=scale, n_layers=len(layers), legacy=legacy)
         self._fuse_stem()
+        self._fuse_tail1x1()
 
     def _fuse_stem(self):
         if not self.fuse_stem or len(self.ops) < 2:
@@ -791,6 +797,46 @@
                               in_dtype=self.in_dtype, name=a["name"] + "+" + b["name"].split(".")[-1], lane=0,
                               mfma_flops=a["mfma_flops"] + b["mfma_flops"])]
         self.layer_out[0] = None
+
+    def _fuse_tail1x1(self):
+        if not self.fuse_cv1:
+            return
+        views = lambda o: [o.get(k) for k in ("src0", "src1", "res")] + [t for k in self._LIST_KEYS for t in (o.get(k) or [])]
+        i = 0
+        while i < len(self.ops):
+            a = self.ops[i]
+            i += 1
+            mid = a.get("dst")
+            if (a["kind"] != L.OP_CONV or a["ksize"] != 3 or a.get("src1") is not None or a["src0"].up or a.get("res") is not None
+                    or a.get("out_f32") or a.get("ksplit") or a.get("dst_scale", 1) != 1 or a.get("tail1_c") or a.get("mid_c")):
+                continue
+            cin, cout = a["src0"].C, a.get("cout", mid.C)
+            if cout > 256 or cout % 32 or cin % 64 or cout != mid.C or mid.cmap is not None or a["src0"].cmap is not None:
+                continue
+            if self.B * a["OH"] * a["OW"] < self.tail1_min_pixels:
+                continue
+            if self.latency and self.split_factors(3, a["stride"], cin, cin, cout, a["OH"], a["OW"]) != (1, 1):
+                continue
+            if mid.coff or any(o is not a and o.get("dst") is not None and o["dst"].buf == mid.buf for o in self.ops):
+                continue
+            readers = [o for o in self.ops if any(t is not None and t.buf == mid.buf for t in views(o))]
+            if len(readers) != 1:
+                continue
+            b = readers[0]
+            s0 = b.get("src0")
+            if (b["kind"] != L.OP_CONV or b["ksize"] != 1 or b["stride"] != 1 or b.get("src1") is not None or b.get("res") is not None
+                    or b.get("out_f32") or b.get("ksplit") or b.get("dst_scale", 1) != 1 or b.get("mid_c") or b.get("tail1_c")
+                    or s0 is None or s0.buf != mid.buf or s0.coff != mid.coff or s0.C != mid.C or s0.up or s0.cmap is not None
+                    or b.get("cout", b["dst"].C) > 256 or b.get("cout", b["dst"].C) != b["dst"].C or b["dst"].C % 8 or b["dst"].ld % 8
+                    or b["dst"].coff % 8 or b.get("lane", 0) != a.get("lane", 0) or b.get("join") or self.ops[i] is not b):
+                continue
+            fused = dict(a, dst=b["dst"], wkey2=b["wkey"], tail1_c=b["dst"].C, tail1_act=b["act"],
+                         name=a["name"] + "+" + ".".join(b["name"].split(".")[-2:]), mfma_flops=a["mfma_flops"] + b["mfma_flops"])
+            self.ops[i - 1:i + 1] = [fused]
+            self.buf_bytes[mid.buf] = 16
+            for n, t in enumerate(self.layer_out):
+                if isinstance(t, T) and t.buf == mid.buf:
+                    self.layer_out[n] = None
 
     _VIEW_KEYS = ("src0", "src1", "dst", "res")
     _LIST_KEYS = ("box", "cls", "msk")
@@ -866,9 +912,10 @@
         if o["kind"] != L.OP_CONV or self.f32_mode:
             return None
         s0, s1, d, r = o["src0"], o.get("src1"), o["dst"], o.get("res")
-        return (self.B, o["H"], o["W"], s0.C, s0.ld, int(s0.up), s1.C if s1 else 0, s1.ld if s1 else 0, int(s1.up) if s1 else 0,
-                o.get("cout", d.C), d.ld, o["ksize"], o["stride"], int(r is not None), r.ld if r is not None else 0,
-                o.get("out_f32", 0), o.get("dst_scale", 1), o.get("act", 0), o.get("ksplit", 0))
+        sg = (self.B, o["H"], o["W"], s0.C, s0.ld, int(s0.up), s1.C if s1 else 0, s1.ld if s1 else 0, int(s1.up) if s1 else 0,
+              o.get("cout", d.C), d.ld, o["ksize"], o["stride"], int(r is not None), r.ld if r is not None else 0,
+              o.get("out_f32", 0), o.get("dst_scale", 1), o.get("act", 0), o.get("ksplit", 0))
+        return sg + (o["tail1_c"], o["tail1_act"]) if o.get("tail1_c") else sg
 
     def c_ops(self):
         arr = (L.Op * len(self.ops))()
@@ -882,7 +929,7 @@
             o.up1 = int(bool(d.get("src1") and d["src1"].up))
             o.dst, o.res = v(d.get("dst")), v(d.get("res"))
             o.ksize, o.stride, o.pad = d.get("ksize", 0), d.get("stride", 0), d.get("pad", 0)
-            o.act, o.out_f32 = d.get("act", 0), d.get("out_f32", 0)
+            o.act, o.out_f32 = d.get("act", 0) | (d.get("tail1_act", 0) << 1), d.get("out_f32", 0)
             o.dst_scale, o.dst_dy, o.dst_dx = d.get("dst_scale", 1), d.get("dst_dy", 0), d.get("dst_dx", 0)
             if "wkey" in d:
                 w = self.wrecs[d["wkey"]]
@@ -893,6 +940,8 @@
                 assert w.w_off >= 0, "pack weights before serialising"
                 o.w2_off, o.b2_off = w.w_off, w.b_off
             o.mid_c = d.get("mid_c", 0)
+            if d.get("tail1_c"):
+                o.mid_c = d.get("cout", 0)
             for j, k in enumerate(d.get("wkeys", [])):
                 w = self.wrecs[k]
                 assert w.w_off >= 0, "pack weights before serialising"
diff --git a/include/bsyolo.h b/include/bsyolo.h
--- a/include/bsyolo.h
+++ b/include/bsyolo.h
@@ -112,6 +112,12 @@
 
 int bsy_conv2d(const void* x, int ldx, int B, int H, int W, int C1, const void* w, const float* b, void* y, int ldy,
                int C2, int ksize, int stride, int act, const void* res, int ldr, int y_f32, bsy_stream stream);
+int bsy_conv2d_tail1(const void* x, int ldx, int B, int H, int W, int C1, const void* w, const float* b, int C2, int stride, int act,
+                     const void* w2, const float* b2, int C3, int act2, void* y, int ldy, const void* res, int ldr, int cfg,
+                     bsy_stream stream);
+int bsy_conv2d_tail1_configs(const void* x, int ldx, int B, int H, int W, int C1, const void* w, const float* b, int C2, int stride,
+                             int act, const void* w2, const float* b2, int C3, int act2, void* y, int ldy, const void* res, int ldr,
+                             int* out, int max_out);
 int bsy_conv2d_f32(const float* x, int ldx, int B, int H, int W, int C1, const float* w, const float* b, float* y, int ldy,
                    int C2, int ksize, int stride, int act, const float* res, int ldr, int impl, bsy_stream stream);
 int bsy_conv2d_f32x(const float* x, int ldx, int B, int H, int W, int C1, const void* w_hi, const void* w_lo, int k_pad,
```
